# adahbingee/pais-mvs

Measured on AMD Instinct MI355X. Metric: refined+expanded patches/sec, higher is better.
Workload: dtype f64

## Files before the change

include/pais_hip.h:

```cpp
#ifndef PAIS_HIP_H
#define PAIS_HIP_H

#include <stdint.h>
#include <stddef.h>

#ifdef __cplusplus
extern "C" {
#endif

#define PAIS_MAX_LEVELS 16
#define PAIS_MAX_VIS    64
#define PAIS_MAX_PARTICLES 128

#define PAIS_TYPE_SEED   0
#define PAIS_TYPE_EXPAND 1

typedef struct pais_config {
    int32_t cellSize;
    int32_t patchRadius;
    int32_t patchSize;
    int32_t minCamNum;
    double  textureVariation;
    double  visibleCorrelation;
    double  minCorrelation;
// ... 92 lines not shown

int  pais_ctx_create(const pais_config *cfg, int num_cams, const pais_camera_desc *cams,
                     int device, uint64_t pso_seed, pais_ctx **out);
int  pais_ctx_set_config(pais_ctx *ctx, const pais_config *cfg);
int  pais_ctx_set_neighbor_radius(pais_ctx *ctx, double neighbor_radius);
void pais_ctx_destroy(pais_ctx *ctx);

int  pais_fitness_batch(pais_ctx *ctx, int n_states, const pais_patch_state *states,
                        int n_evals, const int32_t *state_index, const double *particles,
                        double *out);

#define PAIS_COST_OK          0
#define PAIS_COST_BACKFACING  1
#define PAIS_COST_OFF_IMAGE   2
#define PAIS_COST_WINDOW      3
#define PAIS_COST_OVERFLOW    4
#define PAIS_COST_ALL_MASKED  5
#define PAIS_PIX_COUNTED      0
#define PAIS_PIX_MASKED       1
#define PAIS_PIX_OVERFLOW     2
#define PAIS_PIX_NONE         3

typedef struct pais_cost_detail {
    double  fitness;
    double  sum_weight;
    double  sum_weighted_sad;
    double  pt[2];
    int32_t outcome, nx, ny;
    int32_t live_pixels;
    int32_t overflow_pixel;
    int32_t overflow_cam;
    int32_t ref_pos, _pad;
} pais_cost_detail;

int  pais_fitness_detail(pais_ctx *ctx, int n_states, const pais_patch_state *states,
                         int n_evals, const int32_t *state_index, const double *particles,
                         pais_cost_detail *out, double *weight, double *avg_sad, int8_t *pixel_code,
                         double *colour, double *homographies, int cam_stride);
int  pais_get_detail_stats(pais_ctx *ctx, double *kernel_ms, int64_t *launches, int64_t *evals, int reset);
size_t pais_sizeof_cost_detail(void);

int  pais_refine_batch(pais_ctx *ctx, int n, const pais_candidate *cands, pais_patch_result *out);
int  pais_refine_batch_view(pais_ctx *ctx, int n, const pais_candidate *cands, const pais_patch_result **view);
int  pais_refine_batch_begin(pais_ctx *ctx, int n, const pais_candidate *cands);
int  pais_refine_batch_end(pais_ctx *ctx, const pais_patch_result **view);

typedef struct pais_pso_run_info {
    double  range_l[3], range_u[3];
    double  init[3];
    double  ray[3];
    int32_t run;
    int32_t ref_cam, lod, num_cam;
    int32_t n_particles, max_iteration;
    int32_t iterations;
    int32_t _pad;
    int32_t cam_idx[PAIS_MAX_VIS];
} pais_pso_run_info;

typedef struct pais_pso_iter {
    double  gbest_fitness, gbest[3];
    double  iw;
    double  dispersion, velocity;
    int32_t g_idx, iteration, ended, _pad;
} pais_pso_iter;

int  pais_pso_trace_shape(pais_ctx *ctx, int n, const pais_candidate *cands, int *rows_per_run, int *particles_per_row);
int  pais_pso_trace(pais_ctx *ctx, int n, const pais_candidate *cands, int max_runs, pais_patch_result *out,
                    pais_pso_run_info *runs, pais_pso_iter *iters, double *particles);
int  pais_get_trace_stats(pais_ctx *ctx, double *kernel_ms, int64_t *launches, int64_t *evals, int reset);
size_t pais_sizeof_pso_run_info(void);
size_t pais_sizeof_pso_iter(void);

int  pais_refine_batch_open(pais_ctx *ctx, int n, const pais_candidate *cands, int iterations);
int  pais_refine_batch_enqueue(pais_ctx *ctx, int iterations);
int  pais_ctx_fork_lane(pais_ctx *parent, pais_ctx **lane);
int  pais_ctx_set_round_hint(pais_ctx *ctx, int n_round);

int  pais_refine_batch_device(pais_ctx *ctx, int n, const pais_candidate *d_cands,
                              pais_patch_result *d_out, int max_num_cam, int has_seeds);
size_t pais_record_wire_bytes(int max_num_cam);
int  pais_pack_records(int n, const pais_patch_result *recs, int max_num_cam, void *wire);
int  pais_unpack_records(int n, const void *wire, int max_num_cam, pais_patch_result *recs);
int  pais_pack_records_device(pais_ctx *ctx, int n, const pais_patch_result *d_recs, int max_num_cam, void *d_wire);

#define PAIS_WIRE_MAGIC 0x50414953u
#define PAIS_WIRE_RC_RING_RETRY 1
#define PAIS_WIRE_HEADER_BYTES 64
int  pais_refine_batch_device_async(pais_ctx *ctx, int n, const pais_candidate *d_cands,
                                    pais_patch_result *d_out, int max_num_cam, int has_seeds);
int  pais_wire_header_device(pais_ctx *ctx, int rank, int count, int host_rc, uint32_t user_word, void *d_header);
int  pais_ctx_batch_status(pais_ctx *ctx);

void *pais_ctx_stream(pais_ctx *ctx);
int  pais_ctx_synchronize(pais_ctx *ctx);

typedef struct pais_kernel_stats {
    double   pso_ms;
    double   begin_ms;
    double   after_ms;
    int64_t  pso_launches;
    int64_t  pso_evals;
    int64_t  pso_patches;
    double   pso_algorithmic_bytes;
    double   ncc_algorithmic_bytes;
    int64_t  ncc_tables;
    double   eval_ms;
    int64_t  eval_launches;
    double   eval2_ms;
    int64_t  eval2_launches;
    int64_t  eval2_evals;
    double   eval2_algorithmic_bytes;
    int64_t  tile_launches;
    double   eval2_busy_ms;
    int64_t  ring_launches;
    double   ring_ms;
    int64_t  ring_evals;
    double   ring_algorithmic_bytes;
    int64_t  ring_fallbacks;
} pais_kernel_stats;
int  pais_get_kernel_stats(pais_ctx *ctx, pais_kernel_stats *out, int reset);
int  pais_ctx_set_fine_timing(pais_ctx *ctx, int on);

int  pais_neighbor_count(pais_ctx *ctx, int n, const double *centers, double radius, int32_t *counts, double *kernel_ms);

typedef struct pais_view_state {
    double  center[3];
    double  normal[3];
    int32_t ref_cam, lod, num_cam, _pad;
    int32_t cam_idx[PAIS_MAX_VIS];
} pais_view_state;

#define PAIS_VIEW_KEEP         0
#define PAIS_VIEW_REGION       1
#define PAIS_VIEW_BACKFACING   2
#define PAIS_VIEW_CORRELATION  3
#define PAIS_VIEW_DROP_SAMPLE  1
#define PAIS_VIEW_DROP_MINCAM  2

typedef struct pais_view_result {
    double  correlation;
    double  region_ratio[PAIS_MAX_VIS];
    int32_t dropped, max_idx, num_kept, _pad;
    int32_t reason[PAIS_MAX_VIS];
    int32_t kept_idx[PAIS_MAX_VIS];
} pais_view_result;

int  pais_ncc_batch(pais_ctx *ctx, int n, const pais_view_state *states, pais_view_result *out, double *tables, int stride);
int  pais_get_ncc_stats(pais_ctx *ctx, double *kernel_ms, int64_t *launches, int64_t *states, int reset);
size_t pais_sizeof_view_state(void);
size_t pais_sizeof_view_result(void);

typedef struct pais_loaded_patch {
    double  center[3], normalS[2], fitness, correlation;
    int32_t num_cam, _pad;
    int32_t cam_idx[PAIS_MAX_VIS];
} pais_loaded_patch;
int  pais_load_state_batch(pais_ctx *ctx, int n, const pais_loaded_patch *in, pais_patch_result *out);
int  pais_get_load_stats(pais_ctx *ctx, double *kernel_ms, int64_t *launches, int64_t *patches, int reset);
size_t pais_sizeof_loaded_patch(void);

uint32_t pais_rand31(uint64_t seed, uint64_t key, uint32_t run, uint32_t k);
uint64_t pais_child_key(uint64_t parent_key, int cam, int cx, int cy);

const char *pais_last_error(void);
size_t pais_sizeof_config(void);
size_t pais_sizeof_camera_desc(void);
// ... 8 lines not shown
```

pais_mvs_amd/_lib.py:

```python
from __future__ import annotations

import ctypes as C
import os

from . import build as _build

MAX_LEVELS = 16
MAX_VIS = 64


class Config(C.Structure):
    _fields_ = [
        ("cellSize", C.c_int32), ("patchRadius", C.c_int32), ("patchSize", C.c_int32), ("minCamNum", C.c_int32),
        ("textureVariation", C.c_double), ("visibleCorrelation", C.c_double), ("minCorrelation", C.c_double),
        ("maxFitness", C.c_double), ("lodRatio", C.c_double),
        ("minLOD", C.c_int32), ("maxLOD", C.c_int32), ("maxCellPatchNum", C.c_int32), ("_pad0", C.c_int32),
        ("reduceNormalRange", C.c_double),
        ("adaptiveDistanceEnable", C.c_int32), ("adaptiveDifferenceEnable", C.c_int32),
        ("adaptiveGradientEnable", C.c_int32), ("_pad1", C.c_int32),
        ("distWeighting", C.c_double), ("diffWeighting", C.c_double), ("gradientWeighting", C.c_double),
        ("neighborRadius", C.c_double), ("neighborRadiusScalar", C.c_double), ("minRegionRatio", C.c_double),
        ("depthRangeScalar", C.c_double),
        ("particleNum", C.c_int32), ("maxIteration", C.c_int32), ("expansionStrategy", C.c_int32), ("_pad2", C.c_int32),
    ]
# ... 78 lines not shown
                ("velocity", C.c_double), ("g_idx", C.c_int32), ("iteration", C.c_int32), ("ended", C.c_int32), ("_pad", C.c_int32)]


class View(C.Structure):
    _fields_ = [("R", C.c_double * 9), ("T", C.c_double * 3), ("focal", C.c_double * 2), ("pp", C.c_double * 2)]


RENDER_DISC, RENDER_POINT, RENDER_CULL_BACK, RENDER_MAX_POINT_SIZE = 0, 1, 1, 64
CLOUD_MAX_K, KNN_SKIP_SAME_INDEX = 32, 1


class Lens(C.Structure):
    _fields_ = [("focal", C.c_double * 2), ("pp", C.c_double * 2), ("k", C.c_double), ("model", C.c_int32), ("_pad", C.c_int32)]


LENS_MEASURED_TO_IDEAL, LENS_IDEAL_TO_MEASURED = 0, 1


class KernelStats(C.Structure):
    _fields_ = [("pso_ms", C.c_double), ("begin_ms", C.c_double), ("after_ms", C.c_double),
                ("pso_launches", C.c_int64), ("pso_evals", C.c_int64), ("pso_patches", C.c_int64),
                ("pso_algorithmic_bytes", C.c_double), ("ncc_algorithmic_bytes", C.c_double),
                ("ncc_tables", C.c_int64), ("eval_ms", C.c_double), ("eval_launches", C.c_int64),
                ("eval2_ms", C.c_double), ("eval2_launches", C.c_int64), ("eval2_evals", C.c_int64),
                ("eval2_algorithmic_bytes", C.c_double), ("tile_launches", C.c_int64), ("eval2_busy_ms", C.c_double), ("ring_launches", C.c_int64),
                ("ring_ms", C.c_double), ("ring_evals", C.c_int64), ("ring_algorithmic_bytes", C.c_double), ("ring_fallbacks", C.c_int64)]


_lib = None


def load(build_if_needed: bool = True):
    global _lib
    if _lib is not None:
        return _lib
    path = os.environ.get("PAIS_LIB_PATH") or _build.LIB
    if path != _build.LIB:
        build_if_needed = False
    if int(os.environ.get("WORLD_SIZE", "1")) > 1 or os.environ.get("PAIS_NO_BUILD"):
        build_if_needed = False
    if build_if_needed and _build.needs_build():
        try:
            _build.build()
        except Exception as e:
            if not os.path.exists(path):
                raise RuntimeError("libpais_hip.so is missing and could not be built: %s" % e)
    if not os.path.exists(path):
        raise RuntimeError("libpais_hip.so not found at %s -- run `python -m pais_mvs_amd.build`" % path)
    L = C.CDLL(path)
    L.pais_last_error.restype = C.c_char_p
    for n in ("pais_sizeof_config", "pais_sizeof_camera_desc", "pais_sizeof_candidate", "pais_sizeof_patch_result",
              "pais_sizeof_view_state", "pais_sizeof_view_result", "pais_sizeof_cost_detail",
              "pais_sizeof_pso_run_info", "pais_sizeof_pso_iter", "pais_sizeof_loaded_patch"):
        getattr(L, n).restype = C.c_size_t
    assert L.pais_sizeof_config() == C.sizeof(Config), (L.pais_sizeof_config(), C.sizeof(Config))
    assert L.pais_sizeof_camera_desc() == C.sizeof(CameraDesc)
    assert L.pais_sizeof_candidate() == C.sizeof(Candidate)
    assert L.pais_sizeof_patch_result() == C.sizeof(PatchResult), (L.pais_sizeof_patch_result(), C.sizeof(PatchResult))
    assert L.pais_sizeof_view_state() == C.sizeof(ViewState), (L.pais_sizeof_view_state(), C.sizeof(ViewState))
    assert L.pais_sizeof_view_result() == C.sizeof(ViewResult), (L.pais_sizeof_view_result(), C.sizeof(ViewResult))
    assert L.pais_sizeof_cost_detail() == C.sizeof(CostDetail), (L.pais_sizeof_cost_detail(), C.sizeof(CostDetail))
    assert L.pais_sizeof_pso_run_info() == C.sizeof(PsoRunInfo), (L.pais_sizeof_pso_run_info(), C.sizeof(PsoRunInfo))
    assert L.pais_sizeof_pso_iter() == C.sizeof(PsoIter), (L.pais_sizeof_pso_iter(), C.sizeof(PsoIter))
    assert L.pais_sizeof_loaded_patch() == C.sizeof(LoadedPatch), (L.pais_sizeof_loaded_patch(), C.sizeof(LoadedPatch))
    L.pais_ctx_create.restype = C.c_int
    L.pais_ctx_create.argtypes = [C.POINTER(Config), C.c_int, C.POINTER(CameraDesc), C.c_int, C.c_uint64,
                                  C.POINTER(C.c_void_p)]
    L.pais_ctx_set_config.argtypes = [C.c_void_p, C.POINTER(Config)]
    L.pais_ctx_set_neighbor_radius.argtypes = [C.c_void_p, C.c_double]
    L.pais_ctx_destroy.argtypes = [C.c_void_p]
    L.pais_ctx_destroy.restype = None
    L.pais_ctx_stream.restype = C.c_void_p
    L.pais_ctx_stream.argtypes = [C.c_void_p]
    L.pais_ctx_synchronize.argtypes = [C.c_void_p]
    L.pais_fitness_batch.argtypes = [C.c_void_p, C.c_int, C.POINTER(PatchState), C.c_int, C.POINTER(C.c_int32),
                                     C.POINTER(C.c_double), C.POINTER(C.c_double)]
    L.pais_refine_batch.argtypes = [C.c_void_p, C.c_int, C.POINTER(Candidate), C.POINTER(PatchResult)]
    L.pais_refine_batch_device.argtypes = [C.c_void_p, C.c_int, C.c_void_p, C.c_void_p, C.c_int, C.c_int]
    L.pais_refine_batch_begin.argtypes = [C.c_void_p, C.c_int, C.POINTER(Candidate)]
    L.pais_refine_batch_open.argtypes = [C.c_void_p, C.c_int, C.POINTER(Candidate), C.c_int]
    L.pais_refine_batch_enqueue.argtypes = [C.c_void_p, C.c_int]
    L.pais_ctx_set_round_hint.argtypes = [C.c_void_p, C.c_int]
    L.pais_refine_batch_end.argtypes = [C.c_void_p, C.POINTER(C.POINTER(PatchResult))]
    L.pais_ctx_fork_lane.argtypes = [C.c_void_p, C.POINTER(C.c_void_p)]
    L.pais_get_kernel_stats.argtypes = [C.c_void_p, C.POINTER(KernelStats), C.c_int]
    L.pais_ctx_set_fine_timing.argtypes = [C.c_void_p, C.c_int]
    L.pais_neighbor_count.argtypes = [C.c_void_p, C.c_int, C.POINTER(C.c_double), C.c_double, C.POINTER(C.c_int32), C.POINTER(C.c_double)]
    L.pais_ncc_batch.argtypes = [C.c_void_p, C.c_int, C.POINTER(ViewState), C.POINTER(ViewResult), C.POINTER(C.c_double), C.c_int]
    L.pais_fitness_detail.argtypes = [C.c_void_p, C.c_int, C.POINTER(PatchState), C.c_int, C.POINTER(C.c_int32),
                                      C.POINTER(C.c_double), C.POINTER(CostDetail), C.POINTER(C.c_double), C.POINTER(C.c_double),
                                      C.POINTER(C.c_int8), C.POINTER(C.c_double), C.POINTER(C.c_double), C.c_int]
    L.pais_pso_trace.argtypes = [C.c_void_p, C.c_int, C.POINTER(Candidate), C.c_int, C.POINTER(PatchResult), C.c_void_p, C.c_void_p,
                                 C.POINTER(C.c_double)]
    L.pais_pso_trace_shape.argtypes = [C.c_void_p, C.c_int, C.POINTER(Candidate), C.POINTER(C.c_int), C.POINTER(C.c_int)]
    L.pais_get_trace_stats.argtypes = [C.c_void_p, C.POINTER(C.c_double), C.POINTER(C.c_int64), C.POINTER(C.c_int64), C.c_int]
    L.pais_get_detail_stats.argtypes = [C.c_void_p, C.POINTER(C.c_double), C.POINTER(C.c_int64), C.POINTER(C.c_int64), C.c_int]
    L.pais_get_ncc_stats.argtypes = [C.c_void_p, C.POINTER(C.c_double), C.POINTER(C.c_int64), C.POINTER(C.c_int64), C.c_int]
    L.pais_load_state_batch.argtypes = [C.c_void_p, C.c_int, C.POINTER(LoadedPatch), C.POINTER(PatchResult)]
    L.pais_get_load_stats.argtypes = [C.c_void_p, C.POINTER(C.c_double), C.POINTER(C.c_int64), C.POINTER(C.c_int64), C.c_int]
    L.pais_cloud_nearest.argtypes = [C.c_int, C.c_int, C.POINTER(C.c_double), C.c_int, C.POINTER(C.c_double),
                                     C.POINTER(C.c_int32), C.POINTER(C.c_double), C.POINTER(C.c_double)]
    L.pais_cloud_knn.argtypes = [C.c_int, C.c_int, C.c_int, C.c_int, C.POINTER(C.c_double), C.c_int, C.POINTER(C.c_double),
                                 C.POINTER(C.c_int32), C.POINTER(C.c_double), C.POINTER(C.c_double)]
    L.pais_cloud_outlier_rule.argtypes = [C.c_int, C.c_int, C.POINTER(C.c_int32), C.POINTER(C.c_double), C.c_double,
                                          C.POINTER(C.c_double), C.POINTER(C.c_double), C.POINTER(C.c_uint8)]
    L.pais_cloud_normals.argtypes = [C.c_int, C.POINTER(C.c_double), C.POINTER(C.c_double)]
    L.pais_cloud_launches.restype = C.c_int64
    L.pais_cloud_launches.argtypes = []
    L.pais_cloud_last_error.restype = C.c_char_p
    L.pais_sizeof_view.restype = C.c_size_t
    assert L.pais_sizeof_view() == C.sizeof(View), (L.pais_sizeof_view(), C.sizeof(View))
    L.pais_cloud_render.argtypes = [C.c_int, C.c_int, C.c_int, C.c_int, C.POINTER(C.c_double), C.POINTER(C.c_double),
                                    C.POINTER(C.c_double), C.c_double, C.c_int, C.POINTER(View), C.c_int, C.c_int,
                                    C.POINTER(C.c_double), C.POINTER(C.c_int32), C.POINTER(C.c_double)]
    L.pais_render_launches.restype = C.c_int64
    L.pais_render_launches.argtypes = []
    L.pais_render_last_error.restype = C.c_char_p
    L.pais_render_last_counts.restype = None
    L.pais_render_last_counts.argtypes = [C.POINTER(C.c_int64)] * 4
    L.pais_sizeof_lens.restype = C.c_size_t
    assert L.pais_sizeof_lens() == C.sizeof(Lens), (L.pais_sizeof_lens(), C.sizeof(Lens))
    for n in ("pais_undistort_points", "pais_distort_points"):
        getattr(L, n).argtypes = [C.c_int, C.POINTER(Lens), C.c_int64, C.POINTER(C.c_double), C.POINTER(C.c_double),
                                  C.POINTER(C.c_uint8), C.POINTER(C.c_double)]
    L.pais_undistort_image.argtypes = [C.c_int, C.POINTER(Lens), C.c_int, C.c_void_p, C.c_int, C.c_int, C.c_int64, C.c_void_p,
                                       C.c_void_p, C.POINTER(C.c_int64), C.POINTER(C.c_double)]
    L.pais_undistort_launches.restype = C.c_int64
    L.pais_undistort_launches.argtypes = []
    L.pais_undistort_last_error.restype = C.c_char_p
    L.pais_rand31.restype = C.c_uint32
    L.pais_rand31.argtypes = [C.c_uint64, C.c_uint64, C.c_uint32, C.c_uint32]
    L.pais_child_key.restype = C.c_uint64
    L.pais_child_key.argtypes = [C.c_uint64, C.c_int, C.c_int, C.c_int]
    _lib = L
    return L


def check(rc: int, what: str = ""):
    if rc != 0:
        raise RuntimeError("%s failed (%d): %s" % (what or "pais call", rc, load().pais_last_error().decode()))
```

pais_mvs_amd/context.py:

```python
from __future__ import annotations

import ctypes as C
import math
from typing import List, Sequence

import numpy as np

from . import _lib
from .camera import Camera
from .config import MvsConfig


def camera_desc(cam: Camera, with_edges: bool, keep: list) -> "_lib.CameraDesc":
    d = _lib.CameraDesc()
    d.focal[:] = list(map(float, cam.focal))
    d.principle_point[:] = list(map(float, cam.principle_point))
    d.rotation[:] = cam.rotation.ravel().tolist()
    d.translation[:] = cam.translation.tolist()
    d.center[:] = cam.center.tolist()
    d.KR[:] = cam.KR.ravel().tolist()
    d.KT[:] = cam.KT.tolist()
    d.optical_normal[:] = cam.optical_normal.tolist()
    d.max_lod = cam.max_lod
    for l, img in enumerate(cam.pyramid):
        img = np.ascontiguousarray(img, dtype=np.uint8)
        keep.append(img)
        d.level_width[l] = img.shape[1]
        d.level_height[l] = img.shape[0]
        d.level_stride[l] = img.strides[0]
        d.level_image[l] = img.ctypes.data
        if with_edges and cam.edge_pyramid:
            e = np.ascontiguousarray(cam.edge_pyramid[l], dtype=np.float64)
            keep.append(e)
            d.level_edge[l] = e.ctypes.data
    return d


def normal_to_spherical(n) -> List[float]:
    return [math.acos(float(n[2])), math.atan2(float(n[1]), float(n[0]))]


class Context:

    def __init__(self, cfg: MvsConfig, cameras: Sequence[Camera], device: int = 0, seed: int = 42):
        self.L = _lib.load()
        self.cfg = cfg
        self.cameras = list(cameras)
        self._keep: list = []
        n = len(self.cameras)
        descs = (_lib.CameraDesc * n)()
        for i, cam in enumerate(self.cameras):
            descs[i] = camera_desc(cam, bool(cfg.adaptiveGradientEnable), self._keep)
        self._c_cfg = cfg.to_c()
        h = C.c_void_p()
        _lib.check(self.L.pais_ctx_create(C.byref(self._c_cfg), n, descs, device, seed, C.byref(h)), "pais_ctx_create")
        self.h = h
        self._keep.clear()

    def close(self):
        if getattr(self, "h", None):
            self.L.pais_ctx_destroy(self.h)
            self.h = None

    def __del__(self):
        try:
            self.close()
        except Exception:
            pass

    def set_config(self, cfg: MvsConfig):
        c_cfg = cfg.to_c()
        _lib.check(self.L.pais_ctx_set_config(self.h, C.byref(c_cfg)), "pais_ctx_set_config")
        self.cfg = cfg
        self._c_cfg = c_cfg

    def set_neighbor_radius(self, r: float):
        _lib.check(self.L.pais_ctx_set_neighbor_radius(self.h, float(r)))

    def fitness_batch(self, states: Sequence["_lib.PatchState"], state_index: Sequence[int], particles) -> np.ndarray:
        ns = len(states)
        arr = (_lib.PatchState * ns)(*states)
        idx = np.ascontiguousarray(state_index, dtype=np.int32)
        pts = np.ascontiguousarray(particles, dtype=np.float64).reshape(-1, 3)
        assert len(idx) == len(pts)
        out = np.empty(len(idx), dtype=np.float64)
        _lib.check(self.L.pais_fitness_batch(self.h, ns, arr, len(idx), idx.ctypes.data_as(C.POINTER(C.c_int32)),
                                             pts.ctypes.data_as(C.POINTER(C.c_double)),
                                             out.ctypes.data_as(C.POINTER(C.c_double))), "pais_fitness_batch")
        return out

    def refine_batch(self, cands: Sequence["_lib.Candidate"]):
        n = len(cands)
        arr = (_lib.Candidate * n)(*cands)
        out = (_lib.PatchResult * n)()
        _lib.check(self.L.pais_refine_batch(self.h, n, arr, out), "pais_refine_batch")
        return out

    def ncc_batch(self, states: Sequence["_lib.ViewState"], tables: bool = False) -> "NccBatch":
        n = len(states)
        arr = (_lib.ViewState * max(n, 1))(*states)
        out = (_lib.ViewResult * max(n, 1))()
        stride = max([int(s.num_cam) for s in states] + [2])
        tab = np.zeros((n, stride, stride), dtype=np.float64) if tables else None
        tp = tab.ctypes.data_as(C.POINTER(C.c_double)) if tables else None
        _lib.check(self.L.pais_ncc_batch(self.h, n, arr, out, tp, stride), "pais_ncc_batch")
        return NccBatch([int(s.num_cam) for s in states], out, tab)

    def load_state_batch(self, patches: Sequence["_lib.LoadedPatch"]):
        n = len(patches)
        arr = (_lib.LoadedPatch * max(n, 1))(*patches)
        out = (_lib.PatchResult * max(n, 1))()
        _lib.check(self.L.pais_load_state_batch(self.h, n, arr, out), "pais_load_state_batch")
        return out

    def load_stats(self, reset: bool = False):
        ms, launches, np_ = C.c_double(), C.c_int64(), C.c_int64()
        _lib.check(self.L.pais_get_load_stats(self.h, C.byref(ms), C.byref(launches), C.byref(np_), 1 if reset else 0))
        return ms.value, launches.value, np_.value

    def fitness_detail(self, states: Sequence["_lib.PatchState"], state_index: Sequence[int], particles, colours: bool = False,
                       homographies: bool = False) -> "CostDetail":
        ns = len(states)
        arr = (_lib.PatchState * max(ns, 1))(*states)
        idx = np.ascontiguousarray(state_index, dtype=np.int32)
        pts = np.ascontiguousarray(particles, dtype=np.float64).reshape(-1, 3)
        assert len(idx) == len(pts)
        n, S = len(idx), int(self.cfg.patchSize)
        K = max([int(s.num_cam) for s in states] + [1])
        rec = (_lib.CostDetail * max(n, 1))()
        weight = np.zeros((n, S, S), dtype=np.float64)
        avg_sad = np.zeros((n, S, S), dtype=np.float64)
        code = np.zeros((n, S, S), dtype=np.int8)
        col = np.zeros((n, K, S, S), dtype=np.float64) if colours else None
        hom = np.zeros((n, K, 9), dtype=np.float64) if homographies else None
        dp = lambda a: a.ctypes.data_as(C.POINTER(C.c_double)) if a is not None else None
        _lib.check(self.L.pais_fitness_detail(self.h, ns, arr, n, idx.ctypes.data_as(C.POINTER(C.c_int32)), dp(pts), rec, dp(weight),
                                              dp(avg_sad), code.ctypes.data_as(C.POINTER(C.c_int8)), dp(col), dp(hom), K),
                   "pais_fitness_detail")
        num_cam = [int(states[i].num_cam) for i in idx.tolist()]
        return CostDetail(rec, n, weight, avg_sad, code, col, hom, num_cam, int(self.cfg.patchRadius))

    def pso_trace(self, cands: Sequence["_lib.Candidate"], max_runs: int = 1, particles: bool = False) -> "PsoTrace":
        n = len(cands)
        arr = (_lib.Candidate * max(n, 1))(*cands)
        rows, npart = C.c_int(0), C.c_int(0)
        _lib.check(self.L.pais_pso_trace_shape(self.h, n, arr, C.byref(rows), C.byref(npart)), "pais_pso_trace_shape")
        R, N = rows.value, npart.value
        out = (_lib.PatchResult * max(n, 1))()
        run_info = np.zeros((n, max(int(max_runs), 1)), dtype=PSO_RUN_INFO_DTYPE)
        iters = np.zeros((n, max(int(max_runs), 1), R), dtype=PSO_ITER_DTYPE)
        parts = np.zeros((n, max(int(max_runs), 1), R, N, 11), dtype=np.float64) if particles else None
        pp = parts.ctypes.data_as(C.POINTER(C.c_double)) if parts is not None else None
        _lib.check(self.L.pais_pso_trace(self.h, n, arr, int(max_runs), out, run_info.ctypes.data_as(C.c_void_p),
                                         iters.ctypes.data_as(C.c_void_p), pp), "pais_pso_trace")
        return PsoTrace(out, n, run_info, iters, parts)

    def trace_stats(self, reset: bool = False):
        ms, launches, ne = C.c_double(), C.c_int64(), C.c_int64()
        _lib.check(self.L.pais_get_trace_stats(self.h, C.byref(ms), C.byref(launches), C.byref(ne), 1 if reset else 0))
        return ms.value, launches.value, ne.value

    def detail_stats(self, reset: bool = False):
        ms, launches, ne = C.c_double(), C.c_int64(), C.c_int64()
        _lib.check(self.L.pais_get_detail_stats(self.h, C.byref(ms), C.byref(launches), C.byref(ne), 1 if reset else 0))
        return ms.value, launches.value, ne.value

    def ncc_stats(self, reset: bool = False):
        ms, launches, nst = C.c_double(), C.c_int64(), C.c_int64()
        _lib.check(self.L.pais_get_ncc_stats(self.h, C.byref(ms), C.byref(launches), C.byref(nst), 1 if reset else 0))
        return ms.value, launches.value, nst.value

    def kernel_stats(self, reset: bool = False) -> "_lib.KernelStats":
        st = _lib.KernelStats()
        _lib.check(self.L.pais_get_kernel_stats(self.h, C.byref(st), 1 if reset else 0))
        return st


def make_candidate(center, normal, cam_idx, key: int, ptype: int, normalS=None) -> "_lib.Candidate":
    c = _lib.Candidate()
    c.center[:] = [float(v) for v in center]
# ... 196 lines not shown
```

pais_mvs_amd/csrc/pais_capi.hip:

```cpp
#include <hip/hip_runtime.h>
#include <limits.h>
#include <math.h>
#include <stdarg.h>
#include <stddef.h>
#include <stdio.h>
#include <stdlib.h>
#include <string.h>

#include <string>
#include <utility>
#include <vector>
#include <algorithm>

#include "../../include/pais_hip.h"
#include "../../include/pais_test_hooks.h"
#include "pais_dev.hpp"
#include "pais_host.hpp"
#include "pais_internal.h"

static thread_local std::string g_err;
static int fail(const char *what, hipError_t e)
{
    char buf[512];
    snprintf(buf, sizeof(buf), "%s: %s", what, hipGetErrorString(e));
    g_err = buf;
    return -2;
}
static int fail_msg(const char *what)
{
    g_err = what;
    return -1;
}
__attribute__((format(printf, 1, 2))) static int fail_fmt(const char *fmt, ...)
{
    char buf[512];
    va_list ap;
    va_start(ap, fmt);
    vsnprintf(buf, sizeof(buf), fmt, ap);
    va_end(ap);
    return fail_msg(buf);
}
#define HIPCHK(call)                                   \
    do {                                               \
        hipError_t e__ = (call);                       \
        if (e__ != hipSuccess) return fail(#call, e__); \
    } while (0)

struct EventPair {
    hipEvent_t a, b;
};

struct pais_ctx;
struct Timed {
    pais_ctx *ctx = nullptr;
    hipStream_t st = nullptr;
    std::vector<EventPair> *into = nullptr;
    EventPair e{nullptr, nullptr};
    bool on = false;
    int begin(pais_ctx *c, hipStream_t s, std::vector<EventPair> *v);
    int end();
};
struct LaunchStats {
    double ms = 0;
    int64_t launches = 0, items = 0;
};
struct TimedLaunch {
    pais_ctx *ctx;
    EventPair e{nullptr, nullptr};
    explicit TimedLaunch(pais_ctx *c) : ctx(c) {}
    TimedLaunch(TimedLaunch &&o) noexcept : ctx(o.ctx), e(o.e) { o.e = EventPair{nullptr, nullptr}; }
    ~TimedLaunch();
    int begin();
    int end();
    void collect(LaunchStats &s, int64_t items, int64_t launches = 1);
};
struct TraceOut {
    pais_launch::TraceSink sink{nullptr, nullptr, nullptr, 1, 1};
    std::vector<TimedLaunch> passes;
    int64_t launches = 0;
};
struct PassPlan {
    struct Slice { int lo, hi, parts; pais_launch::BatchView v; pais_launch::TraceSink trace; };
    pais_launch::BatchView all{};
    int nSl = 0, S = 1, afterGrid = 0, itNext = 0;
    bool useIter = false, useTile = false, useRing = false, hasSeeds = false;
    bool usePre = false;
    int ringCUs = 0;
    Slice sl[16];
    int *cnt = nullptr, *nextCnt = nullptr;
    const pais_candidate *d_cands = nullptr;
    Timed tp;
    TraceOut *trace = nullptr;
};

struct pais_ctx {
    int device = 0;
    hipStream_t stream = nullptr;
    int numCUs = 256;
    size_t ldsLimit = 64 * 1024;
    DevScene sc;
    DevBuf<DevCamera> d_cams;
    DevBuf<uint8_t> d_img;
    DevBuf<PaisImgT> d_imgF;
    DevBuf<double> d_edge;
    bool edgesOnTheFly = false;
    DevBuf<double> d_gauss;
    size_t imgBytes = 0, edgeBytes = 0;
    std::vector<int> camMaxLod;
    DevBuf<pais_candidate> d_cands;
    DevBuf<pais_patch_result> d_recs;
    PinBuf<pais_candidate> h_cands;
    PinBuf<pais_patch_result> h_recs;
    DevBuf<double> d_hp;
    DevBuf<double> d_ratios;
    DevBuf<int> d_counters;
    unsigned passSerial = 0;
    bool countersDirty = false;
    DevBuf<unsigned char> d_evalBlocks;
    DevBuf<unsigned char> d_win;
    DevBuf<int> d_active;
    DevBuf<unsigned long long> d_stat;
    unsigned long long *stat = nullptr;
    PinBuf<int> h_counters;
    DevBuf<unsigned char> d_psoStates;
    long splitAbove = 0;
    int psoMinPer = 64;
    int evalParts = 0;
    double partFill = 0.5;
    int psoStreams = 2;
    pais_launch::TileOpts tile;
    int arithLiteral = 0;
    bool tileVerify = false;
    bool tileDebug = false;
    int tileMode = 1;
    long tileAbove = 512;
    std::vector<hipStream_t> sub;
    std::vector<hipEvent_t> subDone;
    hipEvent_t forkEv = nullptr;
    DevBuf<pais_patch_state> d_states;
    DevBuf<int32_t> d_idx;
    DevBuf<double> d_particles, d_out;
    DevBuf<pais_view_state> d_vStates;
    DevBuf<pais_view_result> d_vOut;
    DevBuf<double> d_vTables, d_vHp;
    LaunchStats ncc;
    DevBuf<pais_loaded_patch> d_lIn;
    DevBuf<pais_patch_result> d_lOut;
    LaunchStats load;
    DevBuf<pais_patch_state> d_dStates;
    DevBuf<int32_t> d_dIdx;
    DevBuf<double> d_dParticles, d_dWeight, d_dSad, d_dColour, d_dH;
    DevBuf<pais_cost_detail> d_dRec;
    DevBuf<int8_t> d_dCode;
    LaunchStats detail;
    DevBuf<pais_candidate> d_tCands;
    DevBuf<pais_patch_result> d_tRecs;
    DevBuf<pais_pso_run_info> d_tRuns;
    DevBuf<pais_pso_iter> d_tIters;
    DevBuf<double> d_tParts;
    DevBuf<unsigned long long> d_tStat;
    LaunchStats trace;
    DevBuf<double> d_nbC;
    DevBuf<int32_t> d_nbN;
    bool fineTiming = false;
    std::vector<EventPair> evPso, evBegin, evAfter, evEval, evEval2;
    std::vector<EventPair> evFree;
    double psoMs = 0, beginMs = 0, afterMs = 0, evalMs = 0, eval2Ms = 0;
    hipEvent_t refEv = nullptr;
    std::vector<std::pair<float, float>> eval2Intervals;
    int64_t psoLaunches = 0, evalLaunches = 0, eval2Launches = 0, tileLaunches = 0, ringLaunches = 0;
    pais_ctx *parent = nullptr;
    std::vector<pais_ctx *> lanes;
    int openBatch = -1;
    double ringPerCam = 1843.0;
    int ringMode = 1;
    int preMode = 1;
    DevBuf<double> d_pre;
    DevBuf<unsigned> d_ring;
    DevBuf<unsigned> d_ringCtl;
    PinBuf<unsigned> h_ringCtl;
    DevBuf<int> d_arrive;
    bool ringUsed = false;
    bool ringSuppressed = false;
    bool ringSuppressOnce = false;
    int ringPendingN = 0;
    double ringTimeoutMs = 10000.0;
    long ringSeedAbove = 0;
    size_t ringMaxBytes = (size_t)512 << 20;
    int64_t ringFallbacks = 0;
    std::vector<EventPair> evRing;
    double ringMs = 0;
    PassPlan plan;
    bool planDone = true;
    int roundHint = 0;
};
// ... 812 lines not shown
    if (itEnd > P.all.maxIt + 1) itEnd = P.all.maxIt + 1;
    if (P.useRing) {
        if (P.itNext == 0 && itEnd > 0) {
            const unsigned long long ticks = (unsigned long long)(ctx->ringTimeoutMs * 1e5);
            auto ring = [&](int phase) {
                return pais_launch::pso_ring(sc, P.all, ctx->d_ring, ctx->d_ringCtl, ctx->d_arrive, ctx->stat, P.ringCUs, phase, ticks);
            };
            HIPCHK(ring(0));
            Timed te;
            if (te.begin(ctx, ctx->stream, &ctx->evRing)) return -2;
            HIPCHK(ring(1));
            if (te.end()) return -2;
            HIPCHK(hipMemcpyAsync(ctx->h_ringCtl, ctx->d_ringCtl, PAIS_RING_CTL_BYTES * PAIS_RINGS, hipMemcpyDeviceToHost, ctx->stream));
            ctx->ringUsed = true;
            ctx->evalLaunches++;
            ctx->eval2Launches++;
            ctx->ringLaunches++;
            P.itNext = P.all.maxIt + 1;
        }
        return 0;
    }
    TimedLaunch tpass(ctx);
    const bool timePass = P.trace && itEnd > P.itNext;
    if (timePass && tpass.begin()) return -2;
    for (int it = P.itNext; it < itEnd; ++it) {
        for (int k = 0; k < P.nSl; ++k) {
            const PassPlan::Slice &q = P.sl[k];
            Timed te;
            if (te.begin(ctx, q.v.stream, P.useIter ? &ctx->evEval : &ctx->evEval2)) return -2;
            if (P.useIter)
                HIPCHK(pais_launch::pso_iter(sc, q.v, ctx->d_active, P.cnt + 2, q.lo, q.hi, ctx->stat, it, 0, q.parts));
            else if (P.useTile) {
                HIPCHK(pais_launch::pso_tile(sc, q.v, ctx->tile, ctx->tileDebug ? ctx->stat + 8 : nullptr));
                HIPCHK(pais_launch::pso_eval(sc, q.v, ctx->tileVerify ? 2 : 1, ctx->stat + 18));
            } else if (ctx->arithLiteral)
                HIPCHK(pais_launch::pso_eval_literal(sc, q.v));
            else
                HIPCHK(pais_launch::pso_eval(sc, q.v, 0, nullptr));
            if (te.end()) return -2;
            ctx->evalLaunches++;
            if (!P.useIter) ctx->eval2Launches++;
            if (P.useTile) ctx->tileLaunches++;
            if (P.trace) {
                HIPCHK(pais_launch::pso_step_trace(sc, q.v, ctx->stat, q.trace));
                P.trace->launches++;
            } else if (!P.useIter)
                HIPCHK(pais_launch::pso_step(sc, q.v, ctx->stat));
        }
    }
    if (timePass) {
        if (tpass.end()) return -2;
        P.trace->passes.push_back(std::move(tpass));
    }
    if (itEnd > P.itNext) P.itNext = itEnd;
    return 0;
}

static int pass_join(pais_ctx *ctx, PassPlan &P)
{
    for (int sI = 1; sI < P.S; ++sI) {
        bool used = false;
        for (int k = 0; k < P.nSl; ++k) used = used || (P.sl[k].v.stream == ctx->sub[sI - 1]);
        if (!used) continue;
        HIPCHK(hipEventRecord(ctx->subDone[sI - 1], ctx->sub[sI - 1]));
        HIPCHK(hipStreamWaitEvent(ctx->stream, ctx->subDone[sI - 1], 0));
    }
    P.S = 1;
    return 0;
}

static int pass_close(pais_ctx *ctx, PassPlan &P)
{
    const DevScene &sc = ctx->sc;
    for (int k = 0; k < P.nSl; ++k) {
        const PassPlan::Slice &q = P.sl[k];
        if (P.useIter)
            HIPCHK(pais_launch::pso_iter(sc, q.v, ctx->d_active, P.cnt + 2, q.lo, q.hi, ctx->stat, P.all.maxIt + 1, 1, q.parts));
    }
    if (pass_join(ctx, P)) return -2;
    if (P.tp.end()) return -2;
    ctx->psoLaunches++;
    Timed ta;
    if (ta.begin(ctx, ctx->stream, &ctx->evAfter)) return -2;
    HIPCHK(pais_launch::after(sc, P.all.recs, P.all.n, ctx->d_hp, P.afterGrid, P.cnt, ctx->stat, P.all.Kmax, ctx->d_ratios, P.nextCnt, ctx->stream));
    if (ta.end()) return -2;
    return 0;
}

static int batch_setup(pais_ctx *ctx, PassPlan &P, int n, const pais_candidate *d_cands, pais_patch_result *d_out, int max_num_cam, int has_seeds)
{
    HIPCHK(hipSetDevice(ctx->device));
    const DevScene &sc = ctx->sc;
    int Kmax = max_num_cam > 0 ? max_num_cam : sc.numCams;
    if (Kmax > PAIS_MAX_VIS) Kmax = PAIS_MAX_VIS;
    if (Kmax > sc.numCams) Kmax = sc.numCams;
    if (Kmax < 1) Kmax = 1;
    const int Nmax = has_seeds ? sc.cfg.particleNum * 2 : sc.cfg.particleNum;
    const int S2 = sc.cfg.patchSize * sc.cfg.patchSize;
    const int afterGrid = n < 2048 ? n : 2048;
    {
        size_t hpNeed = (size_t)afterGrid * Kmax * S2 * sizeof(double);
        const size_t full = (size_t)2048 * Kmax * S2 * sizeof(double);
        if (hpNeed > ctx->d_hp.bytes && full < ((size_t)1 << 31)) hpNeed = full;
        HIPCHK(ctx->d_hp.reserve(ctx->stream, hpNeed));
    }
    HIPCHK(ctx->d_active.reserve(ctx->stream, sizeof(int) * (size_t)n));
    HIPCHK(ctx->d_evalBlocks.reserve(ctx->stream, pais_launch::eval_block_bytes_host(Kmax) * (size_t)n));
    HIPCHK(ctx->d_win.reserve(ctx->stream, pais_launch::win_bytes_per_candidate(sc) * (size_t)n));
    HIPCHK(ctx->d_psoStates.reserve(ctx->stream, pais_launch::pso_state_bytes_host(Nmax) * (size_t)n));
    HIPCHK(ctx->d_ratios.reserve(ctx->stream, sizeof(double) * PAIS_MAX_VIS * (size_t)n));
    P.all = pais_launch::BatchView{d_out, ctx->d_psoStates, ctx->d_evalBlocks, ctx->d_win, nullptr, n, Nmax, Kmax,
                                   has_seeds ? sc.cfg.maxIteration * 2 : sc.cfg.maxIteration, ctx->stream};
    P.hasSeeds = has_seeds != 0;
    P.afterGrid = afterGrid;
    P.d_cands = d_cands;

    if (ctx->countersDirty) HIPCHK(hipMemsetAsync(ctx->d_counters, 0, sizeof(int) * 8, ctx->stream));
    ctx->countersDirty = true;
    Timed tb;
    if (tb.begin(ctx, ctx->stream, &ctx->evBegin)) return -2;
    HIPCHK(pais_launch::begin(sc, P.all, d_cands, ctx->d_active, ctx->d_counters + 4 * (ctx->passSerial & 1) + 2));
    if (tb.end()) return -2;
    return 0;
}

static int ring_failed(pais_ctx *ctx, int n)
{
    if (!ctx->ringUsed) return 0;
    ctx->ringUsed = false;
    unsigned done = 0, err = 0;
    for (int r = 0; r < PAIS_RINGS; ++r) { done += ctx->h_ringCtl[(PAIS_RING_CTL_BYTES / 4) * r + PAIS_RING_CTL_DONE_WORD]; err |= ctx->h_ringCtl[(PAIS_RING_CTL_BYTES / 4) * r + PAIS_RING_CTL_ERROR_WORD]; }
    if (err == 0 && done == (unsigned)n) return 0;
    ctx->ringFallbacks++;
    if (getenv("PAIS_RING_VERBOSE") || (ctx->ringFallbacks == 1 && ctx->ringTimeoutMs > 0))
        fprintf(stderr, "[pais] k_pso_ring did not complete (error %u, %u of %d runs ended): the batch is re-run with one launch per iteration\n", err, done, n);
    return 1;
}

static int refine_device_once(pais_ctx *ctx, int n, const pais_candidate *d_cands, pais_patch_result *d_out, int max_num_cam, int has_seeds,
                              bool defer = false, TraceOut *trace = nullptr)
{
    PassPlan &P = ctx->plan;
    P.trace = trace;
    ctx->ringUsed = false;
    ctx->ringPendingN = 0;
    int rc = batch_setup(ctx, P, n, d_cands, d_out, max_num_cam, has_seeds);
    int againCount = 0;
    const int maxPass = has_seeds ? (PAIS_MAX_VIS + 2) : 1;
    for (int pass = 0; !rc && pass < maxPass; ++pass) {
        if ((rc = pass_open(ctx, P, pass, againCount)) != 0) break;
        if ((rc = pass_iterations(ctx, P, P.all.maxIt + 1)) != 0) { (void)pass_join(ctx, P); break; }
        if ((rc = pass_close(ctx, P)) != 0) break;
        if (!has_seeds && !ctx->ringUsed) break;
        if (!has_seeds && defer) { ctx->ringPendingN = n; break; }
        if (has_seeds) HIPCHK(hipMemcpyAsync(ctx->h_counters, P.cnt, sizeof(int) * 2, hipMemcpyDeviceToHost, ctx->stream));
        HIPCHK(hipStreamSynchronize(ctx->stream));
        if (ring_failed(ctx, n)) { ctx->roundHint = 0; return 1; }
        if (!has_seeds || ctx->h_counters[1] == 0) break;
        againCount = ctx->h_counters[1];
    }
    ctx->roundHint = 0;
    if (rc) return rc;
    ctx->countersDirty = false;
    return 0;
}

static int rerun_without_ring(pais_ctx *ctx, int n, const pais_candidate *d_cands, pais_patch_result *d_out, int max_num_cam, int has_seeds,
                              bool defer, int hint)
{
    ctx->ringSuppressed = true;
    ctx->countersDirty = true;
    ctx->roundHint = hint;
    const int rc = refine_device_once(ctx, n, d_cands, d_out, max_num_cam, has_seeds, defer);
    ctx->ringSuppressed = false;
    return rc;
}

static int refine_device(pais_ctx *ctx, int n, const pais_candidate *d_cands, pais_patch_result *d_out, int max_num_cam, int has_seeds, bool defer)
{
    const int hint = ctx->roundHint;
    const int rc = refine_device_once(ctx, n, d_cands, d_out, max_num_cam, has_seeds, defer);
    return rc == 1 ? rerun_without_ring(ctx, n, d_cands, d_out, max_num_cam, has_seeds, defer, hint) : rc;
}

extern "C" int pais_refine_batch_device(pais_ctx *ctx, int n, const pais_candidate *d_cands, pais_patch_result *d_out,
                                        int max_num_cam, int has_seeds)
{
    if (!ctx || n < 0) return fail_msg("pais_refine_batch_device: bad argument");
    if (n == 0) return 0;
    if (!d_cands || !d_out) return fail_msg("pais_refine_batch_device: null pointer");
    if (ctx->openBatch >= 0) return fail_msg("pais_refine_batch_device: a batch is open on this context");
    return refine_device(ctx, n, d_cands, d_out, max_num_cam, has_seeds, false);
}

extern "C" int pais_refine_batch_device_async(pais_ctx *ctx, int n, const pais_candidate *d_cands, pais_patch_result *d_out,
                                              int max_num_cam, int has_seeds)
{
    if (!ctx || n < 0) return fail_msg("pais_refine_batch_device_async: bad argument");
    if (n == 0) return 0;
    if (!d_cands || !d_out) return fail_msg("pais_refine_batch_device_async: null pointer");
    if (ctx->openBatch >= 0) return fail_msg("pais_refine_batch_device_async: a batch is open on this context");
    if (ctx->ringSuppressOnce) {
        ctx->ringSuppressOnce = false;
        return rerun_without_ring(ctx, n, d_cands, d_out, max_num_cam, has_seeds, true, ctx->roundHint);
    }
    return refine_device(ctx, n, d_cands, d_out, max_num_cam, has_seeds, true);
}

extern "C" int pais_ctx_batch_status(pais_ctx *ctx)
{
    if (!ctx) return fail_msg("pais_ctx_batch_status: bad argument");
    if (ctx->ringPendingN <= 0) return 0;
    const int n = ctx->ringPendingN;
    ctx->ringPendingN = 0;
    ctx->countersDirty = false;
    if (!ring_failed(ctx, n)) return 0;
    ctx->countersDirty = true;
    ctx->ringSuppressOnce = true;
    return 1;
}

extern "C" int pais_wire_header_device(pais_ctx *ctx, int rank, int count, int host_rc, uint32_t user_word, void *d_header)
{
    if (!ctx || !d_header) return fail_msg("pais_wire_header_device: bad argument");
    HIPCHK(hipSetDevice(ctx->device));
    HIPCHK(pais_launch::wire_header(d_header, ctx->ringPendingN > 0 ? ctx->d_ringCtl : nullptr, ctx->ringPendingN, rank, count, host_rc, user_word, ctx->stream));
    return 0;
}

extern "C" int pais_test_swarm_step(int device, pais_test_swarm *s, double *swarm)
{
    hipError_t e = hipSetDevice(device);
    if (e != hipSuccess) return (int)e;
    return pais_launch::test_swarm_step(s, swarm);
}

extern "C" int pais_ctx_set_round_hint(pais_ctx *ctx, int n_round)
{
    if (!ctx) return fail_msg("pais_ctx_set_round_hint: bad argument");
    ctx->roundHint = n_round > 0 ? n_round : 0;
    return 0;
}

extern "C" int pais_refine_batch_view(pais_ctx *ctx, int n, const pais_candidate *cands, const pais_patch_result **view)
{
    if (!ctx || n < 0) return fail_msg("pais_refine_batch: bad argument");
    if (n == 0) return 0;
    if (!cands || !view) return fail_msg("pais_refine_batch: null pointer");
    int rc = pais_refine_batch_begin(ctx, n, cands);
    if (rc) return rc;
    return pais_refine_batch_end(ctx, view);
}

extern "C" int pais_refine_batch_begin(pais_ctx *ctx, int n, const pais_candidate *cands)
{
    int rc = pais_refine_batch_open(ctx, n, cands, 1 << 20);
    if (rc) return rc;
    rc = pais_refine_batch_enqueue(ctx, 0);
    return rc < 0 ? rc : 0;
}

extern "C" int pais_refine_batch_enqueue(pais_ctx *ctx, int iterations)
{
    if (!ctx) return fail_msg("pais_refine_batch_enqueue: bad argument");
    if (ctx->openBatch < 0) return fail_msg("pais_refine_batch_enqueue: no batch is open on this context");
    if (ctx->planDone) return 1;
    HIPCHK(hipSetDevice(ctx->device));
    PassPlan &P = ctx->plan;
    const int itEnd = iterations > 0 && iterations < P.all.maxIt + 1 - P.itNext ? P.itNext + iterations : P.all.maxIt + 1;
    int rc = pass_iterations(ctx, P, itEnd);
    if (!rc && P.itNext <= P.all.maxIt) return 0;
    if (!rc) rc = pass_close(ctx, P);
    if (rc) { (void)pass_join(ctx, P); ctx->openBatch = -1; ctx->ringUsed = false; return rc; }
    ctx->countersDirty = false;
    HIPCHK(hipMemcpyAsync(ctx->h_recs, ctx->d_recs, sizeof(pais_patch_result) * (size_t)ctx->openBatch, hipMemcpyDeviceToHost, ctx->stream));
    ctx->planDone = true;
    return 1;
}

extern "C" int pais_refine_batch_end(pais_ctx *ctx, const pais_patch_result **view)
{
    if (!ctx || !view) return fail_msg("pais_refine_batch_end: bad argument");
    if (ctx->openBatch < 0) return fail_msg("pais_refine_batch_end: no batch is open on this context");
    if (!ctx->planDone) {
        const int rc = pais_refine_batch_enqueue(ctx, 0);
        if (rc < 0) return rc;
    }
    ctx->openBatch = -1;
    HIPCHK(hipSetDevice(ctx->device));
    HIPCHK(hipStreamSynchronize(ctx->stream));
    if (ring_failed(ctx, ctx->plan.all.n)) {
        const int n = ctx->plan.all.n;
        const int rc = rerun_without_ring(ctx, n, ctx->d_cands, ctx->d_recs, ctx->plan.all.Kmax, 0, false, ctx->roundHint);
        if (rc) return rc;
        HIPCHK(hipMemcpyAsync(ctx->h_recs, ctx->d_recs, sizeof(pais_patch_result) * (size_t)n, hipMemcpyDeviceToHost, ctx->stream));
        HIPCHK(hipStreamSynchronize(ctx->stream));
    }
    *view = ctx->h_recs;
    return 0;
}

extern "C" int pais_refine_batch_open(pais_ctx *ctx, int n, const pais_candidate *cands, int iterations)
{
    if (!ctx || n <= 0 || !cands) return fail_msg("pais_refine_batch_begin: bad argument");
    if (ctx->openBatch >= 0) return fail_msg("pais_refine_batch_begin: a batch is open on this context already");
    HIPCHK(hipSetDevice(ctx->device));
    ctx->ringUsed = false;
    int Kmax = 1, hasSeeds = 0;
    int rc = check_candidates(ctx, "pais_refine_batch", n, cands, Kmax, hasSeeds);
    if (rc) return rc;
    HIPCHK(ctx->d_cands.reserve(ctx->stream, sizeof(pais_candidate) * (size_t)n));
    HIPCHK(ctx->d_recs.reserve(ctx->stream, sizeof(pais_patch_result) * (size_t)n));
    HIPCHK(ctx->h_cands.reserve(ctx->stream, sizeof(pais_candidate) * (size_t)n));
    HIPCHK(ctx->h_recs.reserve(ctx->stream, sizeof(pais_patch_result) * (size_t)n));
    memcpy(ctx->h_cands, cands, sizeof(pais_candidate) * (size_t)n);
    HIPCHK(hipMemcpyAsync(ctx->d_cands, ctx->h_cands, sizeof(pais_candidate) * (size_t)n, hipMemcpyHostToDevice, ctx->stream));
    if (hasSeeds) {
        rc = pais_refine_batch_device(ctx, n, ctx->d_cands, ctx->d_recs, Kmax, 1);
        if (rc) return rc;
        HIPCHK(hipMemcpyAsync(ctx->h_recs, ctx->d_recs, sizeof(pais_patch_result) * (size_t)n, hipMemcpyDeviceToHost, ctx->stream));
        ctx->openBatch = n;
        ctx->planDone = true;
        return 0;
    }
    PassPlan &P = ctx->plan;
    rc = batch_setup(ctx, P, n, ctx->d_cands, ctx->d_recs, Kmax, 0);
    if (!rc) rc = pass_open(ctx, P, 0, 0);
    ctx->roundHint = 0;
    if (!rc && (rc = pass_iterations(ctx, P, iterations > 0 ? iterations : 0)) != 0) (void)pass_join(ctx, P);
    if (rc) { ctx->ringUsed = false; return rc; }
    ctx->openBatch = n;
    ctx->planDone = false;
    return 0;
}

extern "C" int pais_refine_batch(pais_ctx *ctx, int n, const pais_candidate *cands, pais_patch_result *out)
{
    if (n > 0 && !out) return fail_msg("pais_refine_batch: null pointer");
    const pais_patch_result *view = nullptr;
    int rc = pais_refine_batch_view(ctx, n, cands, &view);
    if (rc || n <= 0) return rc;
    memcpy(out, view, sizeof(pais_patch_result) * (size_t)n);
    return 0;
}

extern "C" int pais_pso_trace_shape(pais_ctx *ctx, int n, const pais_candidate *cands, int *rows_per_run, int *particles_per_row)
{
    if (!ctx || n < 0 || !rows_per_run || !particles_per_row) return fail_msg("pais_pso_trace_shape: bad argument");
    if (n > 0 && !cands) return fail_msg("pais_pso_trace_shape: null pointer (cands)");
    int Kmax = 1, hasSeeds = 0;
    const int rc = check_candidates(ctx, "pais_pso_trace_shape", n, cands, Kmax, hasSeeds);
    if (rc) return rc;
    const pais_config &cfg = ctx->sc.cfg;
    *rows_per_run = (hasSeeds ? 2 * cfg.maxIteration : cfg.maxIteration) + 1;
    *particles_per_row = hasSeeds ? 2 * cfg.particleNum : cfg.particleNum;
    return 0;
}

struct TraceScope {
    pais_ctx *ctx;
    unsigned long long *stat;
    bool fine, ringUsed;
    int roundHint, ringPendingN;
    int64_t launches[6];
    explicit TraceScope(pais_ctx *c) : ctx(c)
    {
        stat = c->stat;
        c->stat = c->d_tStat;
        fine = c->fineTiming;
        c->fineTiming = false;
        ringUsed = c->ringUsed;
        ringPendingN = c->ringPendingN;
        roundHint = c->roundHint;
        c->roundHint = 0;
        const int64_t l[6] = {c->psoLaunches, c->evalLaunches, c->eval2Launches, c->tileLaunches, c->ringLaunches, c->ringFallbacks};
        memcpy(launches, l, sizeof(launches));
    }
    ~TraceScope()
    {
        ctx->stat = stat;
        ctx->fineTiming = fine;
        ctx->ringUsed = ringUsed;
        ctx->ringPendingN = ringPendingN;
        ctx->roundHint = roundHint;
        ctx->psoLaunches = launches[0];
        ctx->evalLaunches = launches[1];
        ctx->eval2Launches = launches[2];
        ctx->tileLaunches = launches[3];
        ctx->ringLaunches = launches[4];
        ctx->ringFallbacks = launches[5];
        ctx->plan.trace = nullptr;
    }
};

extern "C" int pais_pso_trace(pais_ctx *ctx, int n, const pais_candidate *cands, int max_runs, pais_patch_result *out,
                              pais_pso_run_info *runs, pais_pso_iter *iters, double *particles)
{
    if (n == 0) return 0;
    if (!ctx) return fail_msg("pais_pso_trace: null pointer (ctx)");
    if (n < 0) return fail_msg("pais_pso_trace: n < 0");
    const char *missing = !cands ? "cands" : !out ? "out" : !runs ? "runs" : !iters ? "iters" : nullptr;
    if (missing) return fail_fmt("pais_pso_trace: null pointer (%s)", missing);
    if (max_runs < 1) return fail_fmt("pais_pso_trace: max_runs %d < 1", max_runs);
    if (ctx->openBatch >= 0) return fail_msg("pais_pso_trace: a stepwise batch is open on this context (pais_refine_batch_open .. _end)");
    int Kmax = 1, hasSeeds = 0;
    int rc = check_candidates(ctx, "pais_pso_trace", n, cands, Kmax, hasSeeds);
    if (rc) return rc;
    HIPCHK(hipSetDevice(ctx->device));
    const pais_config &cfg = ctx->sc.cfg;
    const int rows = (hasSeeds ? 2 * cfg.maxIteration : cfg.maxIteration) + 1;
    const int NP = hasSeeds ? 2 * cfg.particleNum : cfg.particleNum;
    const size_t runRows = (size_t)max_runs * rows;
    const size_t perCand = sizeof(pais_candidate) + sizeof(pais_patch_result) + (size_t)max_runs * sizeof(pais_pso_run_info) +
                           runRows * sizeof(pais_pso_iter) + (particles ? runRows * NP * 11 * sizeof(double) : 0);
    const int chunk = staging_chunk("PAIS_TRACE_STAGING_MB", n, perCand);
    if (!ctx->d_tStat) {
        HIPCHK(ctx->d_tStat.alloc(sizeof(unsigned long long) * 24));
        HIPCHK(hipMemset(ctx->d_tStat, 0, sizeof(unsigned long long) * 24));
    }
    HIPCHK(ctx->d_tCands.reserve(ctx->stream, sizeof(pais_candidate) * (size_t)chunk));
    HIPCHK(ctx->d_tRecs.reserve(ctx->stream, sizeof(pais_patch_result) * (size_t)chunk));
    HIPCHK(ctx->d_tRuns.reserve(ctx->stream, sizeof(pais_pso_run_info) * (size_t)max_runs * chunk));
    HIPCHK(ctx->d_tIters.reserve(ctx->stream, sizeof(pais_pso_iter) * runRows * chunk));
    if (particles) HIPCHK(ctx->d_tParts.reserve(ctx->stream, sizeof(double) * 11 * runRows * NP * chunk));
    TraceScope scope(ctx);
    for (int c0 = 0; c0 < n; c0 += chunk) {
        const int m = std::min(chunk, n - c0);
        const size_t nRuns = (size_t)max_runs * m;
        HIPCHK(hipMemcpyAsync(ctx->d_tCands, cands + c0, sizeof(pais_candidate) * (size_t)m, hipMemcpyHostToDevice, ctx->stream));
        HIPCHK(hipMemsetAsync(ctx->d_tRuns, 0, sizeof(pais_pso_run_info) * nRuns, ctx->stream));
        HIPCHK(hipMemsetAsync(ctx->d_tIters, 0, sizeof(pais_pso_iter) * nRuns * rows, ctx->stream));
        if (particles) HIPCHK(hipMemsetAsync(ctx->d_tParts, 0, sizeof(double) * 11 * nRuns * rows * NP, ctx->stream));
        TraceOut t;
        t.sink = pais_launch::TraceSink{ctx->d_tRuns, ctx->d_tIters, particles ? ctx->d_tParts.p : nullptr, max_runs, rows};
        rc = refine_device_once(ctx, m, ctx->d_tCands, ctx->d_tRecs, Kmax, hasSeeds, false, &t);
        if (rc) {
            (void)hipStreamSynchronize(ctx->stream);
            return rc < 0 ? rc : fail_msg("pais_pso_trace: unexpected ring pass");
        }
        HIPCHK(hipMemcpyAsync(out + c0, ctx->d_tRecs, sizeof(pais_patch_result) * (size_t)m, hipMemcpyDeviceToHost, ctx->stream));
        HIPCHK(hipMemcpyAsync(runs + (size_t)max_runs * c0, ctx->d_tRuns, sizeof(pais_pso_run_info) * nRuns, hipMemcpyDeviceToHost, ctx->stream));
        HIPCHK(hipMemcpyAsync(iters + runRows * c0, ctx->d_tIters, sizeof(pais_pso_iter) * nRuns * rows, hipMemcpyDeviceToHost, ctx->stream));
        if (particles)
            HIPCHK(hipMemcpyAsync(particles + runRows * NP * 11 * c0, ctx->d_tParts, sizeof(double) * 11 * nRuns * rows * NP, hipMemcpyDeviceToHost,
                                  ctx->stream));
        HIPCHK(hipStreamSynchronize(ctx->stream));
        for (TimedLaunch &p : t.passes) p.collect(ctx->trace, 0, 0);
        ctx->trace.launches += t.launches;
        for (int i = 0; i < m; ++i) ctx->trace.items += out[c0 + i].pso_evals;
    }
    return 0;
}

extern "C" int pais_get_trace_stats(pais_ctx *ctx, double *kernel_ms, int64_t *launches, int64_t *evals, int reset)
{
    return read_launch_stats(ctx ? &ctx->trace : nullptr, "pais_get_trace_stats", kernel_ms, launches, evals, reset);
}

static_assert(offsetof(pais_patch_result, imgPoint) == 136 && offsetof(pais_patch_result, key) == 1160 &&
              offsetof(pais_patch_result, type) == 1168 && offsetof(pais_patch_result, cam_idx) == 1200 &&
              offsetof(pais_patch_result, stage) == 1456 && sizeof(pais_patch_result) == 1488, "pais_patch_result layout");
static inline int wire_kw(int max_num_cam)
{
    int k = max_num_cam < 1 ? 1 : (max_num_cam > PAIS_MAX_VIS ? PAIS_MAX_VIS : max_num_cam);
    return (k + 1) & ~1;
}
extern "C" size_t pais_record_wire_bytes(int max_num_cam) { return 208 + 20 * (size_t)wire_kw(max_num_cam); }
extern "C" int pais_pack_records(int n, const pais_patch_result *recs, int max_num_cam, void *wire)
{
    if (n < 0 || (n && (!recs || !wire))) return fail_msg("pais_pack_records: bad argument");
    const int Kw = wire_kw(max_num_cam);
    const size_t WB = pais_record_wire_bytes(max_num_cam);
    for (int i = 0; i < n; ++i) {
        const unsigned char *r = (const unsigned char *)&recs[i];
        unsigned char *w = (unsigned char *)wire + WB * (size_t)i;
        memcpy(w, r, 136);
        memcpy(w + 136, r + 1160, 8);
        memcpy(w + 144, r + 1168, 32);
        memcpy(w + 176, r + 1456, 32);
        memcpy(w + 208, r + 136, 16 * (size_t)Kw);
        memcpy(w + 208 + 16 * (size_t)Kw, r + 1200, 4 * (size_t)Kw);
    }
    return 0;
}
extern "C" int pais_unpack_records(int n, const void *wire, int max_num_cam, pais_patch_result *recs)
{
    if (n < 0 || (n && (!recs || !wire))) return fail_msg("pais_unpack_records: bad argument");
    const int Kw = wire_kw(max_num_cam);
    const size_t WB = pais_record_wire_bytes(max_num_cam);
    for (int i = 0; i < n; ++i) {
        unsigned char *r = (unsigned char *)&recs[i];
        const unsigned char *w = (const unsigned char *)wire + WB * (size_t)i;
        memset(r, 0, sizeof(pais_patch_result));
        memcpy(r, w, 136);
        memcpy(r + 1160, w + 136, 8);
        memcpy(r + 1168, w + 144, 32);
        memcpy(r + 1456, w + 176, 32);
        memcpy(r + 136, w + 208, 16 * (size_t)Kw);
        memcpy(r + 1200, w + 208 + 16 * (size_t)Kw, 4 * (size_t)Kw);
    }
    return 0;
}
extern "C" int pais_pack_records_device(pais_ctx *ctx, int n, const pais_patch_result *d_recs, int max_num_cam, void *d_wire)
{
    if (!ctx || n < 0 || (n && (!d_recs || !d_wire))) return fail_msg("pais_pack_records_device: bad argument");
    HIPCHK(hipSetDevice(ctx->device));
    HIPCHK(pais_launch::pack_records(d_recs, n, wire_kw(max_num_cam), d_wire, ctx->stream));
    return 0;
}

static int collect_stats(pais_ctx *ctx, unsigned long long *st)
{
    HIPCHK(hipStreamSynchronize(ctx->stream));
    if (drain_events(ctx, ctx->evPso, ctx->psoMs)) return -2;
    if (drain_events(ctx, ctx->evBegin, ctx->beginMs)) return -2;
    if (drain_events(ctx, ctx->evAfter, ctx->afterMs)) return -2;
    if (drain_events(ctx, ctx->evEval, ctx->evalMs)) return -2;
    const hipEvent_t ref = ctx->parent ? ctx->parent->refEv : ctx->refEv;
// ... 93 lines not shown
```

pais_mvs_amd/csrc/pais_internal.h:

```cpp
#pragma once
#include <hip/hip_runtime.h>
#include <stdint.h>

#include "../../include/pais_hip.h"

#define PAIS_STAGE_DONE  0
#define PAIS_STAGE_PSO   1
#define PAIS_STAGE_AFTER 2
#define PAIS_STAGE_AFTER2 3
#define PAIS_STAGE_AFTER2_KEEP 4
#define PAIS_STAGE_AFTER2_SAME 7

struct DevCamera {
    double KR[9], KT[3], R[9], T[3], C[3], optN[3], focal[2], pp[2];
    int maxLOD;
    int pad;
    int w[PAIS_MAX_LEVELS], h[PAIS_MAX_LEVELS];
    uint64_t imgOff[PAIS_MAX_LEVELS];
    uint64_t edgeOff[PAIS_MAX_LEVELS];
    double edgeMin[PAIS_MAX_LEVELS], edgeMax[PAIS_MAX_LEVELS];
};

typedef float2 PaisImgT;

struct DevScene {
    pais_config cfg;
    const DevCamera *cams;
    const uint8_t *imgBlob;
    const PaisImgT *imgF;
    const double *edgeBlob;
    const double *gauss;
    double lodScale[PAIS_MAX_LEVELS];
    uint64_t seed;
    int numCams;
    int pad;
};

#ifndef PAIS_RINGS
#define PAIS_RINGS 8
#endif
#ifndef PAIS_ARRIVE_STRIDE
#define PAIS_ARRIVE_STRIDE 16
#endif
#define PAIS_RING_CTL_BYTES 128
#define PAIS_RING_CTL_DONE_WORD 17
#define PAIS_RING_CTL_ERROR_WORD 19

struct pais_test_swarm;
namespace pais_launch {
struct BatchView {
    pais_patch_result *recs;
    unsigned char *states;
    unsigned char *evalBlocks;
    unsigned char *win;
    double *pre;
    int n, Nmax, Kmax, maxIt;
    hipStream_t stream;
    BatchView slice(const DevScene &sc, int lo, int hi, hipStream_t st) const;
};
struct TraceSink {
    pais_pso_run_info *runs;
    pais_pso_iter *iters;
    double *particles;
    int maxRuns, rows;
};
struct TileOpts {
    int stripSteps = 16;
    int noTiles = 0;
};

size_t eval_block_bytes_host(int Kmax);
size_t win_bytes_per_candidate(const DevScene &sc);
size_t pso_state_bytes_host(int Nmax);
size_t pre_bytes_per_candidate(int Nmax, int Kmax);
hipError_t state_blocks(const DevScene &sc, const pais_patch_state *states, int nStates, int Kmax, unsigned char *evalBlocks, void *win,
                        hipStream_t stream);
hipError_t fitness(const DevScene &sc, const pais_patch_state *states, int nStates, const int32_t *idx, const double *particles,
                   double *out, int nEvals, int Kmax, unsigned char *evalBlocks, void *win, int literal, hipStream_t stream);
hipError_t fitness_detail(const DevScene &sc, const int32_t *idx, const double *particles, int nEvals, int Kmax, const unsigned char *evalBlocks,
                          pais_cost_detail *rec, double *weight, double *avgSad, int8_t *code, double *colour, double *H, hipStream_t stream);
hipError_t load_state(const DevScene &sc, const pais_loaded_patch *in, pais_patch_result *recs, int n, uint64_t key0, hipStream_t stream);
hipError_t neighbor_count(const double *centers, int n, double radius, int32_t *counts, hipStream_t stream);
hipError_t expand_image(const uint8_t *img, PaisImgT *out, size_t n, hipStream_t stream);
hipError_t level_edge_minmax(const uint8_t *img, int w, int h, unsigned long long *minmax, hipStream_t stream);
hipError_t pack_records(const pais_patch_result *recs, int n, int Kw, void *wire, hipStream_t stream);
hipError_t wire_header(void *header, const unsigned *ringCtl, int ringN, int rank, int count, int hostRc, uint32_t userWord, hipStream_t stream);

hipError_t begin(const DevScene &sc, const BatchView &v, const pais_candidate *cands, int *activeList, int *activeCount);
hipError_t pso_init(const DevScene &sc, const BatchView &v, int *activeList, int *activeCount);
hipError_t pso_setup0(const DevScene &sc, const BatchView &v);
hipError_t pso_eval(const DevScene &sc, const BatchView &v, int pendingOnly, unsigned long long *verify);
hipError_t pso_eval_literal(const DevScene &sc, const BatchView &v);
bool tile_eligible(int Kmax);
hipError_t pso_tile(const DevScene &sc, const BatchView &v, const TileOpts &o, unsigned long long *dbg);
hipError_t pso_iter(const DevScene &sc, const BatchView &v, const int *activeList, const int *activeCount, int listLo, int listHi,
                    unsigned long long *stat, int L, int finishOnly, int nparts);
hipError_t pso_step(const DevScene &sc, const BatchView &v, unsigned long long *stat);
hipError_t pso_step_trace(const DevScene &sc, const BatchView &v, unsigned long long *stat, const TraceSink &t);
size_t ring_words(int n, int Nmax, int maxIt);
bool pre_ring_ok(int Kmax);
hipError_t pso_ring(const DevScene &sc, const BatchView &v, unsigned *ring, unsigned *ctl, int *arrive, unsigned long long *stat, int waves,
                    int phase, unsigned long long timeoutTicks);
void ring_profile_print();
hipError_t after(const DevScene &sc, pais_patch_result *recs, int n, double *hpScratch, int grid, int *counters,
                 unsigned long long *stat, int Kmax, double *ratios, int *nextCounters, hipStream_t stream);
size_t ncc_lds_bytes(int Kmax);
bool hp_in_lds(const DevScene &sc, int Kmax);
hipError_t ncc_batch(const DevScene &sc, const pais_view_state *states, int n, pais_view_result *out, double *tables, int stride,
                     double *hpScratch, int grid, int Kmax, int hpInLds, hipStream_t stream);
int test_swarm_step(pais_test_swarm *s, double *swarm);
}
```

pais_mvs_amd/csrc/pais_kernels.hip:

```cpp
#include <hip/hip_runtime.h>
#include <stdint.h>
#include <stdlib.h>
#include <string.h>

#include "../../include/pais_hip.h"
#include "../../include/pais_test_hooks.h"
#include "pais_dev.hpp"
#include "pais_internal.h"

using namespace pais;

#ifndef PAIS_NS1_WAVES
#define PAIS_NS1_WAVES 2
#endif
#ifndef PAIS_NS2_WAVES
#define PAIS_NS2_WAVES 3
#endif
#define PAIS_EVAL_BOUNDS(NS) __launch_bounds__(64, (NS) == 1 ? PAIS_NS1_WAVES : PAIS_NS2_WAVES)
#ifndef PAIS_ITER_FREE_REGS_FROM
#define PAIS_ITER_FREE_REGS_FROM 2
#endif
#define PAIS_ITER_BOUNDS(P, NS) __launch_bounds__(64, (P) >= PAIS_ITER_FREE_REGS_FROM ? 1 : ((NS) == 1 ? PAIS_NS1_WAVES : PAIS_NS2_WAVES))
#ifndef PAIS_TWO_PIXELS_MAXK
#define PAIS_TWO_PIXELS_MAXK 6
// ... 1871 lines not shown
        }
        const uint64_t v0 = lane < nwMax ? src[lane] : 0, v1 = lane + 64 < nwMax ? src[lane + 64] : 0;
        const int N = hd->N;
        wave_sync();
        stage_eval_block(smem, src, nwMax, lane, v0, v1);
        wave_sync();
#if PAIS_RING_PROFILE
        asm volatile("s_waitcnt vmcnt(0)" ::: "memory");
#endif
        PAIS_RP_MARK(rpD)
        double f4[4], w4[4];
        int st;
        if (PRE) st = eval_fitness_pre<NS, BYTES, ACCR, true>(sc, ep, cams, Hbuf, cbuf, win + (size_t)c * WS, rec, status0, hv, lane, f4, w4);
        else st = eval_fitness_parts<NS, BYTES, ACCR>(sc, ep, cams, Hbuf, cbuf, win + (size_t)c * WS, p0, p1, p2, lane, 0, 1, f4, w4);
        int old = 0;
        PAIS_RP_MARK(rpE)
        if (lane == 0) {
            cstore(&A.fit[i], st ? DBL_MAX : combine_parts(f4, w4));
            asm volatile("s_waitcnt vmcnt(0)" ::: "memory");
            old = __hip_atomic_fetch_add(&arrive[(size_t)c * PAIS_ARRIVE_STRIDE], 1, __ATOMIC_RELAXED, __HIP_MEMORY_SCOPE_AGENT);
        }
        old = __builtin_amdgcn_readfirstlane(old);
#if PAIS_RING_PROFILE
        {
            const unsigned long long rpF = __builtin_amdgcn_s_memtime();
            if (lane == 0) {
                atomicAdd(&g_ringProf[0], rpB - rpA); atomicAdd(&g_ringProf[1], rpC - rpB); atomicAdd(&g_ringProf[2], rpD - rpC);
                atomicAdd(&g_ringProf[3], rpE - rpD); atomicAdd(&g_ringProf[4], rpF - rpE); atomicAdd(&g_ringProf[6], 1ULL);
            }
        }
        PAIS_RP_MARK(rpG)
#endif
        if (old != N - 1) continue;
        __builtin_amdgcn_s_setprio(3);
        if (lane == 0) cstore(&arrive[(size_t)c * PAIS_ARRIVE_STRIDE], 0);
        wave_sync();
        const int cont = pso_step_wave_ring(sc, recs, c, hd, __builtin_amdgcn_readfirstlane(N), Nmax, smem + (PRE ? eval_block_bytes(Kmax) : 0), stat, lane, ep, cams, crec, preD);
        asm volatile("s_waitcnt vmcnt(0)" ::: "memory");
        wave_sync();
        if (__builtin_amdgcn_readfirstlane(cont)) {
            unsigned base = 0;
            if (lane == 0) base = __hip_atomic_fetch_add(&ctl->tail, (unsigned)N, __ATOMIC_RELAXED, __HIP_MEMORY_SCOPE_AGENT);
            base = (unsigned)__builtin_amdgcn_readfirstlane((int)base);
            if (base + (unsigned)N > cap) {
                if (lane == 0) rstore(&ctl->error, 2u);
                break;
            }
            if (lane < N) rstore(&ring[base + lane], ((unsigned)c << 8) | (unsigned)lane);
        } else if (lane == 0) {
            __hip_atomic_fetch_add(&ctl->done, 1u, __ATOMIC_RELAXED, __HIP_MEMORY_SCOPE_AGENT);
        }
        __builtin_amdgcn_s_setprio(0);
#if PAIS_RING_PROFILE
        {
            const unsigned long long rpH = __builtin_amdgcn_s_memtime();
            if (lane == 0) { atomicAdd(&g_ringProf[5], rpH - rpG); atomicAdd(&g_ringProf[7], 1ULL); }
        }
#endif
    }
}

__global__ __launch_bounds__(64) void k_region_ratio(DevScene sc, const pais_patch_result *recs, int n, int stage, double *ratios, int Kmax)
{
    const int t = blockIdx.x * 64 + threadIdx.x;
    const int c = t / Kmax, k = t - c * Kmax;
    if (c >= n) return;
    const pais_patch_result *P = &recs[c];
    if (P->stage != stage || P->dropped || k >= P->num_cam) return;
    const int LOD = P->lod, refCam = P->ref_cam;
    const DevCamera &rc = sc.cams[refCam];
    const double s = sc.lodScale[LOD];
    const double center[3] = {P->center[0], P->center[1], P->center[2]};
    const double nrm[3] = {P->normal[0], P->normal[1], P->normal[2]};
    const int ci = P->cam_idx[k];
    const double d = -dot3(center, nrm);
    double invH[9], H[9];
    ref_plane_inverse(d, s, rc.KR, rc.KT, nrm, invH);
    patch_homography(ci == refCam, d, s, sc.cams[ci].KR, sc.cams[ci].KT, nrm, invH, H);
    double pt[2];
    cam_project(sc, refCam, center, pt, LOD);
    ratios[(size_t)c * PAIS_MAX_VIS + k] = region_ratio(pt[0], pt[1], sc.cfg.patchRadius, H);
}

template <int PHASE>
__global__ __launch_bounds__(64 * AFTER_WAVES) void k_after(DevScene sc, pais_patch_result *recs, int n, double *hpScratch,
                                                              int *counters, unsigned long long *stat, int Kmax, double *ratios,
                                                              int hpInLds, int *nextCounters)
{
    if (PHASE == 2 && nextCounters && blockIdx.x == 0 && threadIdx.x == 0) {
        nextCounters[0] = 0;
        nextCounters[1] = 0;
        nextCounters[2] = 0;
    }
    extern __shared__ __attribute__((aligned(16))) unsigned char smem[];
    pais_patch_result *st = (pais_patch_result *)smem;
    size_t off = (sizeof(pais_patch_result) + 15) & ~(size_t)15;
    double *table = (double *)(smem + off); off += sizeof(double) * Kmax * Kmax;
    double *Hn = (double *)(smem + off); off += sizeof(double) * 9 * Kmax;
    int *flag = (int *)(smem + off); off += 16;
    const int lane = threadIdx.x & 63, wave = threadIdx.x >> 6;
    const bool lead = threadIdx.x == 0;
    const int S2 = sc.cfg.patchSize * sc.cfg.patchSize;
    double *hp = hpInLds ? (double *)(smem + off) : hpScratch + (size_t)blockIdx.x * Kmax * S2;
    for (int c = blockIdx.x; c < n; c += gridDim.x) {
        const int stg = recs[c].stage;
        if (PHASE == 1 ? (stg != PAIS_STAGE_AFTER) : (stg != PAIS_STAGE_AFTER2 && stg != PAIS_STAGE_AFTER2_KEEP && stg != PAIS_STAGE_AFTER2_SAME))
            continue;
        __syncthreads();
        copy_record(st, &recs[c], threadIdx.x, 64 * AFTER_WAVES);
        __syncthreads();

        const int nccBefore = st->ncc_tables;
        double *rat = ratios + (size_t)c * PAIS_MAX_VIS;
        if (PHASE == 1) {
            const int refBefore = st->ref_cam, lodBefore = st->lod, numBefore = st->num_cam;
            remove_invisible_camera(sc, st, hp, table, Hn, flag, rat, lane, wave);
            const bool removedNone = st->num_cam == numBefore;
            set_reference_camera(sc, st, lane);
            set_depth_and_ray(sc, st, lane);
            set_depth_range(sc, st, lane);
            set_lod(sc, st, lane);

            bool again = false;
            if (st->type != PAIS_TYPE_EXPAND && !st->dropped) {
                const int afterRef = st->ref_cam, afterNum = st->num_cam;
                const int cnt = st->count;
                const bool cond = (st->before_ref != afterRef || st->before_num != afterNum) && (cnt <= st->total_cam_num);
                __syncthreads();
                if (lead) {
                    st->after_ref = afterRef;
                    st->after_num = afterNum;
                    st->count = cnt + 1;
                }
                __syncthreads();
                if (cond) {
                    if (st->num_cam < sc.cfg.minCamNum) {
                        __syncthreads();
                        if (lead) {
                            st->fitness = DBL_MAX;
                            st->priority = DBL_MAX;
                            st->dropped = 1;
                        }
                        __syncthreads();
                    } else {
                        again = true;
                        __syncthreads();
                        if (lead) {
                            st->before_ref = st->ref_cam;
                            st->before_num = st->num_cam;
                            st->stage = PAIS_STAGE_PSO;
                        }
                        __syncthreads();
                    }
                }
            }
            if (!again) {
                set_priority_and_image_point(sc, st, lane);
                __syncthreads();
                if (lead)
                    st->stage = st->dropped ? PAIS_STAGE_DONE
                                            : ((st->ref_cam == refBefore && st->lod == lodBefore)
                                                   ? (removedNone ? PAIS_STAGE_AFTER2_SAME : PAIS_STAGE_AFTER2_KEEP)
                                                   : PAIS_STAGE_AFTER2);
            }
            __syncthreads();
            if (lead && again) atomicAdd(&counters[1], 1);
        } else {
            if (stg == PAIS_STAGE_AFTER2_SAME) {
                if (lead) st->ncc_tables += 1;
            } else {
                remove_invisible_camera(sc, st, hp, table, Hn, flag, rat, lane, wave);
            }
            __syncthreads();
            int finalStage = PAIS_DONE;
            if (!st->dropped) {
                bool off = false;
                const double X[3] = {st->center[0], st->center[1], st->center[2]};
                for (int i = threadIdx.x; i < sc.numCams; i += 64 * AFTER_WAVES) {
                    const DevCamera &cam = sc.cams[i];
                    double pt[2];
                    project_raw(cam.R, cam.T, cam.focal, cam.pp, 1.0, X, pt);
                    if (!in_image_d(pt, cam.w[0], cam.h[0])) {
                        off = true;
                    } else {
                        const int rx = min(cv_round(pt[0]), cam.w[0] - 1), ry = min(cv_round(pt[1]), cam.h[0] - 1);
                        if (sc.imgBlob[cam.imgOff[0] + (size_t)ry * cam.w[0] + rx] == 0) off = true;
                    }
                }
                finalStage = __syncthreads_or(off ? 1 : 0) ? PAIS_DONE_OFF_SCENE : PAIS_DONE_IN_SCENE;
            }
            if (lead) st->stage = finalStage;
        }
        __syncthreads();
        if (lead) {
            atomicAdd(&stat[3], (unsigned long long)(st->ncc_tables - nccBefore));
            atomicAdd(&stat[4], (unsigned long long)(st->ncc_tables - nccBefore) * (unsigned long long)st->total_cam_num);
        }
        __syncthreads();
        copy_record(&recs[c], st, threadIdx.x, 64 * AFTER_WAVES);
    }
}

__global__ __launch_bounds__(64 * AFTER_WAVES) void k_ncc_batch(DevScene sc, const pais_view_state *states, int n,
                                                                  pais_view_result *out, double *tables, int stride,
                                                                  double *hpScratch, int Kmax, int hpInLds)
{
    extern __shared__ __attribute__((aligned(16))) unsigned char smem[];
    pais_view_result *res = (pais_view_result *)smem;
    size_t off = (sizeof(pais_view_result) + 15) & ~(size_t)15;
    double *table = (double *)(smem + off); off += sizeof(double) * Kmax * Kmax;
    double *Hn = (double *)(smem + off); off += sizeof(double) * 9 * Kmax;
    int *flag = (int *)(smem + off); off += 16;
    const int tid = threadIdx.x, lane = tid & 63, wave = tid >> 6;
    const int r = sc.cfg.patchRadius, S = sc.cfg.patchSize, S2 = S * S;
    double *hp = hpInLds ? (double *)(smem + off) : hpScratch + (size_t)blockIdx.x * Kmax * S2;
    for (int s = blockIdx.x; s < n; s += gridDim.x) {
        const pais_view_state *V = &states[s];
        const int K = V->num_cam, LOD = V->lod, refCam = V->ref_cam;
        const double center[3] = {V->center[0], V->center[1], V->center[2]};
        const double nrm[3] = {V->normal[0], V->normal[1], V->normal[2]};
        __syncthreads();
        {
            uint32_t *w = (uint32_t *)res;
            for (int i = tid; i < (int)(sizeof(pais_view_result) / 4); i += 64 * AFTER_WAVES) w[i] = 0;
        }
        for (int i = tid; i < K * K; i += 64 * AFTER_WAVES) table[i] = 0;
        if (tid == 0) *flag = 0;
        if (wave == 0) view_homographies(sc, refCam, sc.lodScale[LOD], V->cam_idx, K, center, nrm, Hn, lane);
        __syncthreads();

        double pt[2];
        cam_project(sc, refCam, center, pt, LOD);
        if (wave == AFTER_WAVES - 1)
            for (int c = lane; c < K; c += 64) res->region_ratio[c] = region_ratio(pt[0], pt[1], r, Hn + 9 * c);

        view_warp_patches(sc, V->cam_idx, K, LOD, Hn, pt[0] - r, pt[1] - r, hp, flag, lane, wave);
        __syncthreads();
        const bool dropSample = *flag != 0;
        if (!dropSample) view_fill_table(hp, K, S2, table, lane, wave);
        __syncthreads();
        if (tid == 0) {
            if (dropSample) {
                res->dropped = PAIS_VIEW_DROP_SAMPLE;
            } else {
                double correlation = 0;
                for (int i = 0; i < K; ++i)
                    for (int j = 0; j < K; ++j) correlation += table[i * K + j];
                correlation /= (double)(K * K - K);
                double maxCorr = -DBL_MAX;
                int maxIdx = 0;
                for (int i = 0; i < K; ++i) {
                    double corrSum = 0;
                    for (int j = 0; j < K; ++j) corrSum += table[i * K + j];
                    if (corrSum >= maxCorr) {
                        maxIdx = i;
                        maxCorr = corrSum;
                    }
                }
                int nn = 0;
                for (int i = 0; i < K; ++i) {
                    const int ci = V->cam_idx[i];
                    const DevCamera &cam = sc.cams[ci];
                    const double dd = nrm[0] * (-cam.optN[0]) + nrm[1] * (-cam.optN[1]) + nrm[2] * (-cam.optN[2]);
                    int why = PAIS_VIEW_KEEP;
                    if (res->region_ratio[i] < sc.cfg.minRegionRatio) why = PAIS_VIEW_REGION;
                    else if (dd < 0) why = PAIS_VIEW_BACKFACING;
                    else if (i != maxIdx && table[maxIdx * K + i] < sc.cfg.minCorrelation) why = PAIS_VIEW_CORRELATION;
                    res->reason[i] = why;
                    if (why == PAIS_VIEW_KEEP) res->kept_idx[nn++] = ci;
                }
                res->correlation = correlation;
                res->max_idx = maxIdx;
                res->num_kept = nn;
                res->dropped = nn < sc.cfg.minCamNum ? PAIS_VIEW_DROP_MINCAM : 0;
            }
        }
        if (tables) {
            double *T = tables + (size_t)s * stride * stride;
            for (int i = tid; i < stride * stride; i += 64 * AFTER_WAVES) {
                const int a = i / stride, b = i - a * stride;
                T[i] = (a < K && b < K) ? table[a * K + b] : 0.0;
            }
        }
        __syncthreads();
        {
            const uint32_t *src = (const uint32_t *)res;
            uint32_t *dst = (uint32_t *)&out[s];
            for (int i = tid; i < (int)(sizeof(pais_view_result) / 4); i += 64 * AFTER_WAVES) dst[i] = src[i];
        }
    }
}

__global__ __launch_bounds__(256) void k_pack_records(const pais_patch_result *recs, int n, int Kw, uint32_t *wire)
{
    const int wordsPerSlot = 52 + 5 * Kw;
    for (size_t t = (size_t)blockIdx.x * 256 + threadIdx.x; t < (size_t)n * wordsPerSlot; t += (size_t)gridDim.x * 256) {
        const int r = (int)(t / wordsPerSlot), w = (int)(t - (size_t)r * wordsPerSlot);
        const uint32_t *src = (const uint32_t *)&recs[r];
        int sw;
        if (w < 34) sw = w;
        else if (w < 36) sw = 290 + (w - 34);
        else if (w < 44) sw = 292 + (w - 36);
        else if (w < 52) sw = 364 + (w - 44);
        else if (w < 52 + 4 * Kw) sw = 34 + (w - 52);
        else sw = 300 + (w - 52 - 4 * Kw);
        wire[t] = src[sw];
    }
}

__global__ __launch_bounds__(64) void k_wire_header(uint32_t *hdr, const RingCtl *ctl, int ringN, int rank, int count, int hostRc, uint32_t userWord)
{
    if (threadIdx.x >= 16) return;
    int rc = hostRc;
    if (rc == 0 && ctl) {
        unsigned done = 0, err = 0;
        for (int r = 0; r < PAIS_RINGS; ++r) { done += ctl[r].done; err |= ctl[r].error; }
        if (err != 0 || done != (unsigned)ringN) rc = PAIS_WIRE_RC_RING_RETRY;
    }
    const uint32_t w[4] = {PAIS_WIRE_MAGIC, (uint32_t)rc, (uint32_t)count, (uint32_t)rank};
    hdr[threadIdx.x] = threadIdx.x < 4 ? w[threadIdx.x] : (threadIdx.x == 4 ? userWord : 0u);
}

__global__ __launch_bounds__(256) void k_expand_image(const uint8_t *img, PaisImgT *out, size_t n)
{
    for (size_t i = (size_t)blockIdx.x * 256 + threadIdx.x; i < n; i += (size_t)gridDim.x * 256) {
        const int a = img[i], b = (i + 1 < n) ? img[i + 1] : 0;
        PaisImgT v;
        v.x = a;
        v.y = b - a;
        out[i] = v;
    }
}
__global__ __launch_bounds__(256) void k_level_edge_minmax(const uint8_t *img, int w, int h, unsigned long long *minmax)
{
    __shared__ unsigned long long red[8];
    const int x = blockIdx.x * 256 + threadIdx.x;
    unsigned long long lo = ~0ULL, hi = 0ULL;
    if (x < w) {
        const int xl = x > 0 ? x - 1 : (w > 1 ? 1 : 0), xr = x < w - 1 ? x + 1 : (w > 1 ? w - 2 : 0);
        for (int r = 0; r < 16; ++r) {
            const int y = blockIdx.y * 16 + r;
            if (y >= h) break;
            const int yu = y > 0 ? y - 1 : (h > 1 ? 1 : 0), yd = y < h - 1 ? y + 1 : (h > 1 ? h - 2 : 0);
            const double gx = (double)img[(size_t)y * w + xr] - (double)img[(size_t)y * w + xl];
            const double gy = (double)img[(size_t)yd * w + x] - (double)img[(size_t)yu * w + x];
            const unsigned long long u = (unsigned long long)__double_as_longlong(sqrt(gx * gx + gy * gy));
            lo = u < lo ? u : lo;
            hi = u > hi ? u : hi;
        }
    }
    for (int s = 32; s >= 1; s >>= 1) {
        const unsigned long long ol = __shfl_xor(lo, s, 64), oh = __shfl_xor(hi, s, 64);
        lo = ol < lo ? ol : lo;
        hi = oh > hi ? oh : hi;
    }
    const int wave = threadIdx.x >> 6;
    if ((threadIdx.x & 63) == 0) {
        red[wave] = lo;
        red[4 + wave] = hi;
    }
    __syncthreads();
    if (threadIdx.x == 0) {
        for (int q = 1; q < 4; ++q) {
            lo = red[q] < lo ? red[q] : lo;
            hi = red[4 + q] > hi ? red[4 + q] : hi;
        }
        if (lo != ~0ULL) atomicMin(&minmax[0], lo);
        atomicMax(&minmax[1], hi);
    }
}

__global__ __launch_bounds__(256) void k_neighbor_count(const double *centers, int n, double radius, int32_t *counts)
{
    __shared__ double tile[256 * 3];
    const int i = blockIdx.x * 256 + threadIdx.x;
    const bool has = i < n;
    const double cx = has ? centers[3 * i] : 0, cy = has ? centers[3 * i + 1] : 0, cz = has ? centers[3 * i + 2] : 0;
    int cnt = 0;
    for (int base = 0; base < n; base += 256) {
        const int m = (n - base) < 256 ? (n - base) : 256;
        __syncthreads();
        for (int t = threadIdx.x; t < 3 * m; t += 256) tile[t] = centers[3 * (size_t)base + t];
        __syncthreads();
        for (int j = 0; j < m; ++j) {
            const double dx = cx - tile[3 * j], dy = cy - tile[3 * j + 1], dz = cz - tile[3 * j + 2];
            double s2 = 0;
            s2 += dx * dx;
            s2 += dy * dy;
// ... 182 lines not shown
    const int groups = (v.Nmax + TILE2_SLOTS - 1) / TILE2_SLOTS;
    return launch<k_pso_tile2<NP>>(grid_for((long)v.n * groups, 65536), dim3(64 * TILE2_WAVES), lds, v.stream, sc, v.states, v.n, v.Nmax, v.Kmax,
                                   (const unsigned char *)v.evalBlocks, eval_block_bytes(v.Kmax), (const WinPix *)v.win,
                                   o.noTiles ? 0 : (int)(lds - fixed), groups, o.stripSteps, dbg);
}
hipError_t pso_tile(const DevScene &sc, const BatchView &v, const TileOpts &o, unsigned long long *dbg)
{
    if (v.Kmax <= 28) return tile_launch<8>(sc, v, o, dbg);
    if (v.Kmax <= 44) return tile_launch<12>(sc, v, o, dbg);
    return tile_launch<16>(sc, v, o, dbg);
}
hipError_t pso_iter(const DevScene &sc, const BatchView &v, const int *activeList, const int *activeCount, int listLo, int listHi,
                    unsigned long long *stat, int L, int finishOnly, int nparts)
{
    if (listHi <= listLo) return hipSuccess;
    return shape_dispatch(sc, v.Kmax, [&](auto ns, auto bytes, auto accr) {
        constexpr int NS = ns;
        constexpr bool BYTES = bytes, ACCR = accr;
        auto go = [&](auto parts) {
            return launch<k_pso_iter<parts, NS, BYTES, ACCR>>(grid_for((long)(listHi - listLo) * (finishOnly ? 1 : v.Nmax * parts), EVAL_GRID_CAP),
                                                              dim3(64), eval_lds_bytes(NS, v.Kmax, ACCR), v.stream, sc, v.states, activeList, activeCount,
                                                              listLo, listHi, v.Nmax, v.Kmax, v.recs, stat, L, finishOnly,
                                                              (const unsigned char *)v.evalBlocks, eval_block_bytes(v.Kmax), (const WinPix *)v.win);
        };
        return nparts == 4 ? go(Int<4>()) : (nparts == 2 ? go(Int<2>()) : go(Int<1>()));
    });
}
static size_t ring_seg_words(int n, int Nmax, int maxIt) { return (size_t)((n + PAIS_RINGS - 1) / PAIS_RINGS) * Nmax * ((size_t)maxIt + 2); }
size_t ring_words(int n, int Nmax, int maxIt) { return ring_seg_words(n, Nmax, maxIt) * PAIS_RINGS; }
hipError_t pso_ring(const DevScene &sc, const BatchView &v, unsigned *ring, unsigned *ctl, int *arrive, unsigned long long *stat, int waves,
                    int phase, unsigned long long timeoutTicks)
{
    const int n = v.n, Nmax = v.Nmax, Kmax = v.Kmax;
    if (Nmax > 64) return hipErrorInvalidValue;
    const size_t words = ring_words(n, Nmax, v.maxIt), seg = ring_seg_words(n, Nmax, v.maxIt);
    if (seg >= 0xFFFFFFF0ull) return hipErrorInvalidValue;
    if (phase == 0) {
        hipError_t e = hipMemsetAsync(ring, 0xFF, words * sizeof(unsigned), v.stream);
        if (e != hipSuccess) return e;
        e = hipMemsetAsync(ctl, 0, sizeof(RingCtl) * PAIS_RINGS, v.stream);
        if (e != hipSuccess) return e;
        e = hipMemsetAsync(arrive, 0, sizeof(int) * PAIS_ARRIVE_STRIDE * (size_t)n, v.stream);
        if (e != hipSuccess) return e;
        return launch<k_ring_init>(dim3((n + 255) / 256), dim3(256), 0, v.stream, v.states, n, Nmax, ring, (unsigned)seg, (RingCtl *)ctl);
    }
    return shape_dispatch(sc, Kmax, [&](auto ns, auto bytes, auto accr) {
        constexpr int NS = ns;
        constexpr bool BYTES = bytes, ACCR = accr;
        const size_t stepBytes = v.pre ? eval_block_bytes(Kmax) + step_lds_bytes(Nmax) : sizeof(double) * (size_t)Nmax * (3 * 4 + 2) + 16;
        size_t per = eval_lds_bytes(NS, Kmax, ACCR);
        if (per < stepBytes) per = stepBytes;
        per = (per + 15) & ~(size_t)15;
        const long resident = (long)waves * (NS == 1 ? 4 * PAIS_NS1_WAVES : 4 * PAIS_NS2_WAVES);
        const unsigned grid = (grid_for((long)n * Nmax, resident) + PAIS_RINGS - 1) / PAIS_RINGS * PAIS_RINGS;
        auto go = [&](auto usePre) {
            return launch<k_pso_ring<NS, BYTES, ACCR, usePre>>(dim3(grid), dim3(64), per, v.stream, sc, v.recs, v.states, n, Nmax, Kmax,
                                                               (const unsigned char *)v.evalBlocks, eval_block_bytes(Kmax), (const WinPix *)v.win, ring,
                                                               (unsigned)seg, (RingCtl *)ctl, arrive, stat, per, timeoutTicks, v.pre);
        };
        return v.pre ? go(Bool<true>()) : go(Bool<false>());
    });
}
hipError_t pso_step(const DevScene &sc, const BatchView &v, unsigned long long *stat)
{
    const size_t lds = v.pre ? eval_block_bytes(v.Kmax) + step_lds_bytes(v.Nmax) : sizeof(double) * (size_t)v.Nmax * (3 * 4 + 2);
    return launch<k_pso_step>(grid_for(v.n, 65536), dim3(64), lds, v.stream, sc, v.recs, v.states, v.n, v.Nmax, stat,
                              (const unsigned char *)v.evalBlocks, eval_block_bytes(v.Kmax), v.pre, v.Kmax);
}
hipError_t pso_step_trace(const DevScene &sc, const BatchView &v, unsigned long long *stat, const TraceSink &t)
{
    if (v.n <= 0) return hipSuccess;
    StepTraceSink sink;
    sink.runs = t.runs;
    sink.iters = t.iters;
    sink.particles = t.particles;
    sink.maxRuns = t.maxRuns;
    sink.rows = t.rows;
    sink.NP = v.Nmax;
    return launch<k_pso_step_trace>(grid_for(v.n, 65536), dim3(64), sizeof(double) * (size_t)v.Nmax * (3 * 4 + 2), v.stream, sc, v.recs, v.states,
                                    v.n, v.Nmax, stat, sink);
}

hipError_t after(const DevScene &sc, pais_patch_result *recs, int n, double *hpScratch, int grid, int *counters,
                 unsigned long long *stat, int Kmax, double *ratios, int *nextCounters, hipStream_t stream)
{
    if (n <= 0) return hipSuccess;
    const int hpInLds = hp_in_lds(sc, Kmax) ? 1 : 0;
    const size_t lds = ncc_scratch_bytes(sizeof(pais_patch_result), Kmax) + (hpInLds ? hp_bytes(sc, Kmax) : 0);
    const dim3 rgrid((unsigned)(((long)n * Kmax + 63) / 64)), block(64 * AFTER_WAVES);
    hipError_t e = launch<k_region_ratio>(rgrid, dim3(64), 0, stream, sc, recs, n, PAIS_STAGE_AFTER, ratios, Kmax);
    if (e == hipSuccess)
        e = launch<k_after<1>>(dim3(grid), block, lds, stream, sc, recs, n, hpScratch, counters, stat, Kmax, ratios, hpInLds, (int *)nullptr);
    if (e == hipSuccess) e = launch<k_region_ratio>(rgrid, dim3(64), 0, stream, sc, recs, n, PAIS_STAGE_AFTER2, ratios, Kmax);
    if (e == hipSuccess)
        e = launch<k_after<2>>(dim3(grid), block, lds, stream, sc, recs, n, hpScratch, counters, stat, Kmax, ratios, hpInLds, nextCounters);
    return e;
}
hipError_t ncc_batch(const DevScene &sc, const pais_view_state *states, int n, pais_view_result *out, double *tables, int stride,
                     double *hpScratch, int grid, int Kmax, int hpInLds, hipStream_t stream)
{
    if (n <= 0) return hipSuccess;
    const size_t lds = ncc_lds_bytes(Kmax) + (hpInLds ? hp_bytes(sc, Kmax) : 0);
    return launch<k_ncc_batch>(dim3(grid), dim3(64 * AFTER_WAVES), lds, stream, sc, states, n, out, tables, stride, hpScratch, Kmax, hpInLds);
}

__global__ __launch_bounds__(64) void k_test_swarm_step(DevScene sc, pais_patch_result *recs, unsigned char *states, int Nmax,
                                                        unsigned long long *stat, int *continues)
{
    extern __shared__ __attribute__((aligned(16))) unsigned char smem0[];
    PsoState *hd = (PsoState *)states;
    const int N = __builtin_amdgcn_readfirstlane(hd->N);
    const int cont = pso_step_wave(sc, recs, 0, hd, N, Nmax, smem0, stat, (int)threadIdx.x);
    if (threadIdx.x == 0) *continues = cont;
}
int test_swarm_step(pais_test_swarm *s, double *swarm)
{
    if (!s || !swarm || s->n < 1 || s->n > 128) return (int)hipErrorInvalidValue;
    const int N = s->n;
    const size_t SB = pso_state_bytes(N), head = (sizeof(PsoState) + 15) & ~(size_t)15;
    unsigned char *host = (unsigned char *)calloc(1, SB);
    if (!host) return (int)hipErrorOutOfMemory;
    PsoState *hd = (PsoState *)host;
    for (int d = 0; d < 3; ++d) {
        hd->rangeL[d] = s->range_l[d];
        hd->rangeU[d] = s->range_u[d];
        hd->ray[d] = d == 2 ? 1.0 : 0.0;
    }
    hd->iw = s->iw;
    hd->gBestFitness = s->gbest_fitness;
    hd->streamBase = s->stream_base;
    hd->gIdx = s->g_idx;
    hd->N = N;
    hd->maxIt = s->max_iteration;
    hd->iteration = s->iteration;
    hd->active = 1;
    hd->run = s->run;
    hd->localK = s->local_k;
    hd->started = s->started;
    hd->K = 3;
    double *arr = (double *)(host + head);
    for (int i = 0; i < N; ++i) {
        for (int a = 0; a < 4; ++a)
            for (int d = 0; d < 3; ++d) arr[(size_t)a * 3 * N + 3 * i + d] = swarm[14 * i + 3 * a + d];
        arr[(size_t)12 * N + i] = swarm[14 * i + 12];
        arr[(size_t)13 * N + i] = swarm[14 * i + 13];
    }
    unsigned char *dev = nullptr;
    const size_t offRec = (SB + 255) & ~(size_t)255, offStat = offRec + ((sizeof(pais_patch_result) + 255) & ~(size_t)255),
                 offCam = offStat + 256, offCont = offCam + ((sizeof(DevCamera) + 255) & ~(size_t)255), total = offCont + 256;
    hipError_t e = hipMalloc((void **)&dev, total);
    if (e == hipSuccess) e = hipMemset(dev, 0, total);
    if (e == hipSuccess) e = hipMemcpy(dev, host, SB, hipMemcpyHostToDevice);
    pais_patch_result rec;
    int cont = 0;
    if (e == hipSuccess) {
        DevScene sc;
        memset(&sc, 0, sizeof(sc));
        sc.cams = (const DevCamera *)(dev + offCam);
        sc.cfg.maxFitness = 10.0;
        sc.numCams = 1;
        e = launch<k_test_swarm_step>(dim3(1), dim3(64), sizeof(double) * (size_t)N * (3 * 4 + 2) + 16, nullptr, sc,
                                      (pais_patch_result *)(dev + offRec), dev, N, (unsigned long long *)(dev + offStat), (int *)(dev + offCont));
    }
    if (e == hipSuccess) e = hipDeviceSynchronize();
    if (e == hipSuccess) e = hipMemcpy(host, dev, SB, hipMemcpyDeviceToHost);
    if (e == hipSuccess) e = hipMemcpy(&rec, dev + offRec, sizeof(rec), hipMemcpyDeviceToHost);
    if (e == hipSuccess) e = hipMemcpy(&cont, dev + offCont, sizeof(int), hipMemcpyDeviceToHost);
    if (e == hipSuccess) {
        for (int i = 0; i < N; ++i) {
            for (int a = 0; a < 4; ++a)
                for (int d = 0; d < 3; ++d) swarm[14 * i + 3 * a + d] = arr[(size_t)a * 3 * N + 3 * i + d];
            swarm[14 * i + 12] = arr[(size_t)12 * N + i];
            swarm[14 * i + 13] = arr[(size_t)13 * N + i];
        }
        s->iw = hd->iw;
        s->gbest_fitness = hd->gBestFitness;
        s->g_idx = hd->gIdx;
        s->iteration = hd->iteration;
// ... 29 lines not shown
```

pais_mvs_amd/csrc/pais_mvs.hip:

```cpp
#include <float.h>
#include <limits.h>
#include <math.h>
#include <stdio.h>
#include <stdlib.h>
#include <string.h>

#include <algorithm>
#include <chrono>
#include <deque>
#include <queue>
#include <new>
#include <string>
#include <unordered_map>
#include <unordered_set>
#include <vector>

#include <dlfcn.h>
#include <hip/hip_runtime.h>

#include "../../include/pais_mvs.h"
#include "../../include/pais_test_hooks.h"
#include "../../include/pais_seed.h"
#include "../../include/pais_feature.h"
#include "../../include/pais_cloud.h"
// ... 780 lines not shown
        for (int i = 0; i < num_cam; i++) {
            const HostCamera &cam = m->cams[cam_idx[i]];
            for (int k = 0; k < 3; ++k) dir[k] = cam.C[k] - center[k];
            double sc = (1.0 / pais::norm3(dir));
            for (int k = 0; k < 3; ++k) dir[k] *= sc;
            for (int k = 0; k < 3; ++k) normal[k] += dir[k];
        }
        double sc = (1.0 / pais::norm3(normal));
        for (int k = 0; k < 3; ++k) r.normal[k] = normal[k] * sc;
        pais::normal2spherical(r.normal, r.normalS);
    } else {
        r.dropped = 1;
    }
    return m->storePatch(r);
}

extern "C" int pais_mvs_add_seed_measured(pais_mvs *m, const double center[3], int num_cam, const int32_t *cam_idx,
                                          const double *img_points, int recenter)
{
    if (!m || !center || num_cam < 0 || num_cam > PAIS_MAX_VIS || (num_cam && (!cam_idx || !img_points)))
        return mfail("pais_mvs_add_seed_measured: bad argument");
    for (int i = 0; i < num_cam; ++i)
        if (cam_idx[i] < 0 || cam_idx[i] >= (int)m->cams.size()) return mfail("pais_mvs_add_seed_measured: bad camera index");
    double c[3] = {center[0], center[1], center[2]};
    if (recenter) {
        double A[3][3] = {{0, 0, 0}, {0, 0, 0}, {0, 0, 0}}, b[3] = {0, 0, 0};
        for (int i = 0; i < num_cam; ++i) {
            const HostCamera &cam = m->cams[cam_idx[i]];
            const double p3[3] = {(img_points[2 * i] - cam.pp[0]) / cam.focal[0] - cam.T[0],
                                  (img_points[2 * i + 1] - cam.pp[1]) / cam.focal[1] - cam.T[1], 1.0 - cam.T[2]};
            double w3[3];
            for (int r = 0; r < 3; ++r) {
                double sacc = 0;
                for (int k = 0; k < 3; ++k) sacc += cam.R[k * 3 + r] * p3[k];
                w3[r] = sacc;
            }
            double n[3] = {w3[0] - cam.C[0], w3[1] - cam.C[1], w3[2] - cam.C[2]};
            const double sc = (1.0 / pais::norm3(n));
            for (int k = 0; k < 3; ++k) n[k] = n[k] * sc;
            const double *cc = cam.C;
            A[0][0] += 1 - n[0] * n[0];
            A[0][1] += -n[0] * n[1];
            A[0][2] += -n[0] * n[2];
            A[1][0] += -n[0] * n[1];
            A[1][1] += 1 - n[1] * n[1];
            A[1][2] += -n[1] * n[2];
            A[2][0] += -n[0] * n[2];
            A[2][1] += -n[1] * n[2];
            A[2][2] += 1 - n[2] * n[2];
            b[0] += (1 - n[0] * n[0]) * cc[0] - n[0] * n[1] * cc[1] - n[0] * n[2] * cc[2];
            b[1] += -n[0] * n[1] * cc[0] + (1 - n[1] * n[1]) * cc[1] - n[1] * n[2] * cc[2];
            b[2] += -n[0] * n[2] * cc[0] - n[1] * n[2] * cc[1] + (1 - n[2] * n[2]) * cc[2];
        }
        double inv[3][3];
        for (int j = 0; j < 3; ++j) {
            double Ac[3][3], e[3] = {0, 0, 0}, col[3];
            for (int r = 0; r < 3; ++r)
                for (int k = 0; k < 3; ++k) Ac[r][k] = A[r][k];
            e[j] = 1.0;
            pais::jacobi_lstsq<3, 3>(Ac, e, col);
            for (int r = 0; r < 3; ++r) inv[r][j] = col[r];
        }
        for (int r = 0; r < 3; ++r) {
            double sacc = 0;
            for (int k = 0; k < 3; ++k) sacc += inv[r][k] * b[k];
            c[r] = sacc;
        }
    }
    const int id = pais_mvs_add_seed(m, c, num_cam, cam_idx);
    if (id >= 0)
        for (int i = 0; i < num_cam; ++i) {
            m->patches[id]->r.imgPoint[i][0] = img_points[2 * i];
            m->patches[id]->r.imgPoint[i][1] = img_points[2 * i + 1];
        }
    return id;
}

#define MHIP(call)                                                                  \
    do {                                                                            \
        hipError_t e__ = (call);                                                    \
        if (e__ != hipSuccess) { g_mvs_err = std::string(#call ": ") + hipGetErrorString(e__); return -2; } \
    } while (0)

static int refine_local(pais_mvs *m, int n, const pais_candidate *c, pais_patch_result *out, int has_seeds,
                        const pais_patch_result **view = nullptr)
{
    if (n <= 0) return 0;
    if (view) *view = out;
    if (m->ctx) {
        int rc = view ? pais_refine_batch_view(m->ctx, n, c, view) : pais_refine_batch(m->ctx, n, c, out);
        if (rc) g_mvs_err = pais_last_error();
        return rc;
    }
    if (m->recordSource) {
        if (m->recordSource(m->recordUser, n, c, out, has_seeds)) return mfail("record source failed");
        return 0;
    }
    return mfail("this driver has neither a GPU context nor a record source");
}

static constexpr size_t kWireHeader = 64;
static int all_gather_host(pais_mvs *m, const void *send, void *recv, size_t bytes)
{
    if (!m->gatherCb) return mfail("no host all-gather installed");
    if (m->gatherCb(m->gatherUser, send, recv, bytes)) return mfail("all-gather callback failed");
    return 0;
}

struct WireHeader { uint32_t magic; int32_t rc; int32_t count; int32_t rank; uint32_t user; };
static bool sharded_transport(const pais_mvs *m) { return m->ctx && (m->nccl || m->emuMode == 2); }
static bool host_transport(const pais_mvs *m) { return !sharded_transport(m) && m->gatherCb != nullptr; }

static int shard_growth_handshake(pais_mvs *m, int localRc)
{
    if (host_transport(m)) {
        std::vector<int> all((size_t)m->world, 0);
        int mine = localRc;
        if (all_gather_host(m, &mine, all.data(), sizeof(int))) return -3;
        for (int r = 0; r < m->world; ++r)
            if (all[(size_t)r] != 0) {
                if (!localRc) g_mvs_err = "sharded batch: rank " + std::to_string(r) + " could not grow its exchange buffers";
                return all[(size_t)r] < 0 ? all[(size_t)r] : -2;
            }
        return 0;
    }
    if (m->emuMode == 2 || !m->nccl) return localRc;
    hipStream_t xs = (hipStream_t)pais_ctx_stream(m->ctx);
    std::string err;
    rccl::Api *a = rccl::api(err);
    if (!a || !m->d_hs) return localRc ? localRc : -2;
    m->h_hs[0] = localRc;
    if (hipMemcpyAsync(m->d_hs, m->h_hs, sizeof(int), hipMemcpyHostToDevice, xs) != hipSuccess) return -2;
    if (a->allGather(m->d_hs, m->d_hsAll, sizeof(int), rccl::kInt8, m->nccl, xs) != 0) return -3;
    if (hipMemcpyAsync(m->h_hs, m->d_hsAll, sizeof(int) * (size_t)m->world, hipMemcpyDeviceToHost, xs) != hipSuccess) return -2;
    if (hipStreamSynchronize(xs) != hipSuccess) return -2;
    for (int r = 0; r < m->world; ++r)
        if (m->h_hs[r] != 0) {
            if (!localRc) g_mvs_err = "sharded batch: rank " + std::to_string(r) + " could not grow its exchange buffers";
            return m->h_hs[r] < 0 ? m->h_hs[r] : -2;
        }
    return 0;
}

static int shard_ensure(pais_mvs *m, pais_mvs::ShardBufs &B, size_t per, size_t slot)
{
    const int world = m->world;
    if (host_transport(m)) {
        const bool grow = per > B.hostC.size() || slot > B.hostS.size() || slot * (size_t)world > B.hostAll.size();
        if (!grow) return 0;
        int rc = 0;
        if (m->injectGrowthFail > 0 && --m->injectGrowthFail == 0) { rc = -2; g_mvs_err = "injected: exchange buffers could not grow"; }
        if (!rc) {
            const size_t cap = per + per / 2 + 64, capS = slot * 3 / 2 + 4096;
            B.hostC.resize(std::max(cap, B.hostC.size()));
            B.hostR.resize(B.hostC.size());
            B.hostS.resize(std::max(capS, B.hostS.size()));
            B.hostAll.resize(std::max(B.hostS.size() * (size_t)world, B.hostAll.size()));
        }
        return shard_growth_handshake(m, rc);
    }
    const bool growShard = per > B.shardCap, growWire = slot * (size_t)world > B.wireCap || slot > B.wireSCap;
    if (!growShard && !growWire && B.packed) return 0;
    hipStream_t xs = (hipStream_t)pais_ctx_stream(m->ctx);
    int rc = 0;
    auto ok = [&](hipError_t e, const char *what) {
        if (e != hipSuccess && !rc) { rc = -2; g_mvs_err = std::string(what) + ": " + hipGetErrorString(e); }
        return e == hipSuccess;
    };
    ok(hipSetDevice(m->device), "hipSetDevice");
    ok(hipDeviceSynchronize(), "hipDeviceSynchronize");
    if (!B.packed) {
// ... 129 lines not shown
    X.per = (n + world - 1) / world;
    X.lo = std::min(m->rank * X.per, n);
    X.cnt = shard_count(m, m->rank, n, X.per);
    X.Kb = 1;
    for (int i = 0; i < n; ++i) X.Kb = std::max(X.Kb, c[i].num_cam);
    X.Kmax = 1;
    for (int j = 0; j < X.cnt; ++j) X.Kmax = std::max(X.Kmax, c[shard_index(m, m->rank, j, n, X.per)].num_cam);
    X.WB = pais_record_wire_bytes(X.Kb);
    X.slot = kWireHeader + X.WB * (size_t)X.per;
    X.t0 = now_ms();
    int rc = shard_ensure(m, B, (size_t)X.per, X.slot);
    if (rc) { X.open = false; return rc; }
    const hipError_t sd = host_transport(m) ? hipSuccess : hipSetDevice(m->device);
    if (m->emuMode == 2 && (rc = emu_fill_blocks(m, X)) != 0) { X.open = false; return rc; }
    if (sd != hipSuccess) g_mvs_err = std::string("hipSetDevice: ") + hipGetErrorString(sd);
    shard_refine_enqueue(m, X, (sd != hipSuccess || preFail) ? -2 : 0);
    rc = shard_exchange(m, X);
    if (rc) X.open = false;
    return rc;
}

static int shard_finish(pais_mvs *m, pais_mvs::ShardXfer &X, pais_patch_result *out)
{
    if (!X.open) return mfail("sharded batch: nothing in flight");
    X.open = false;
    const int world = m->world;
    pais_mvs::ShardBufs &B = *X.B;
    const bool host = host_transport(m);
    const unsigned char *wireAll = host ? B.hostAll.data() : B.h_wireAll;
    for (int attempt = 0;; ++attempt) {
        if (!host) MHIP(hipEventSynchronize(B.done));
        if (m->emuMode == 2 && m->emuLatencyUs > 0) {
            const double t1 = now_ms() + m->emuLatencyUs * 1e-3;
            while (now_ms() < t1) {}
        }
        const int mine = host ? (X.hostRetry ? 1 : 0)
                              : (X.cnt > 0 ? pais_ctx_batch_status(X.lane) : 0);
        bool retry = false;
        for (int r = 0; r < world; ++r) {
            WireHeader hd;
            memcpy(&hd, wireAll + X.slot * (size_t)r, sizeof(hd));
            if (r == 0 && hd.magic == PAIS_WIRE_MAGIC) m->streamAgreed = (hd.user & 1u) != 0;
            const int rcnt = shard_count(m, r, X.n, X.per);
            if (hd.magic != PAIS_WIRE_MAGIC || hd.rank != r || hd.count != rcnt) return mfail("sharded batch: malformed exchange header (ranks disagree on the batch)");
            if (hd.rc == PAIS_WIRE_RC_RING_RETRY) { retry = true; continue; }
            if (hd.rc != 0) {
                if (r != m->rank || g_mvs_err.empty()) g_mvs_err = "sharded batch: rank " + std::to_string(r) + " failed to refine its shard (rc " + std::to_string(hd.rc) + ")";
                return hd.rc < 0 ? hd.rc : -1;
            }
        }
        if (!retry) break;
        if (attempt >= 1) return mfail("sharded batch: a shard did not complete twice");
        X.secondAttempt = true;
        m->st.exchange_retries++;
        if (mine == 1) shard_refine_enqueue(m, X);
        else if (!host && X.lane != m->ctx) MHIP(hipEventRecord(B.packed, (hipStream_t)pais_ctx_stream(X.lane)));
        int rc = shard_exchange(m, X);
        if (rc) return rc;
    }
    m->st.exchange_ms += now_ms() - X.t0;
    for (int r = 0; r < world; ++r) {
        const int rcnt = shard_count(m, r, X.n, X.per);
        const unsigned char *blk = wireAll + X.slot * (size_t)r + kWireHeader;
        if (!m->shardStrided) {
            if (rcnt > 0 && pais_unpack_records(rcnt, blk, X.Kb, out + shard_index(m, r, 0, X.n, X.per))) return mfail(pais_last_error());
        } else {
            for (int j = 0; j < rcnt; ++j)
                if (pais_unpack_records(1, blk + X.WB * (size_t)j, X.Kb, out + shard_index(m, r, j, X.n, X.per))) return mfail(pais_last_error());
        }
    }
    return 0;
}

static void emu_record(pais_mvs *m, int n, const pais_candidate *c, const pais_patch_result *recs)
{
    for (int i = 0; i < n; ++i) {
        auto it = m->emuIndex.find(c[i].key);
        if (it != m->emuIndex.end()) { m->emuRecs[it->second] = recs[i]; continue; }
        m->emuIndex.emplace(c[i].key, (uint32_t)m->emuRecs.size());
        m->emuRecs.push_back(recs[i]);
    }
}

static int refine_any(pais_mvs *m, int n, const pais_candidate *c, pais_patch_result *out, int has_seeds, const pais_patch_result **view)
{
    *view = out;
    if (n <= 0) return 0;
    const int world = m->world;
    if (world <= 1 && !m->nccl && !m->gatherCb) {
        const int rc = refine_local(m, n, c, out, has_seeds, view);
        if (!rc && m->emuMode == 1) emu_record(m, n, c, *view);
        return rc;
    }
    const long wavesPerIter = (long)n * m->cfg.particleNum * (has_seeds ? 2 : 1);
    if (wavesPerIter < (long)m->replicateBelow) {
        m->st.batches_replicated++;
        return refine_local(m, n, c, out, has_seeds, view);
    }
    m->st.batches_sharded++;
    m->results.resize((size_t)n);
    if (!sharded_transport(m) && !host_transport(m)) return mfail("sharded batch: no transport attached");
    int rc = shard_submit(m, m->sx[0], m->sb[0], m->ctx, n, c, has_seeds);
    if (!rc) rc = shard_finish(m, m->sx[0], m->results.data());
    if (rc) return rc;
    *view = m->results.data();
    return 0;
}

extern "C" int pais_mvs_test_inject(pais_mvs *m, int what, int count)
{
    if (!m || count < 0) return mfail("pais_mvs_test_inject: bad argument");
    if (what == 1) m->injectRingRetry = count;
    else if (what == 2) m->injectGrowthFail = count;
    else if (what == 3) m->injectRefineFail = count;
    else return mfail("pais_mvs_test_inject: unknown injection");
    return 0;
}

extern "C" int pais_comm_get_unique_id(pais_unique_id *out)
{
    if (!out) return mfail("pais_comm_get_unique_id: bad argument");
    std::string err;
    rccl::Api *a = rccl::api(err);
    if (!a) return mfail(err.c_str());
    rccl::UniqueId id;
    int nr = a->getUniqueId(&id);
    if (nr != 0) { g_mvs_err = std::string("ncclGetUniqueId: ") + (a->errorString ? a->errorString(nr) : "error"); return -3; }
    memcpy(out->bytes, id.internal, PAIS_UNIQUE_ID_BYTES);
    return 0;
}

extern "C" int pais_mvs_comm_init_rccl(pais_mvs *m, int rank, int world, const pais_unique_id *id)
{
    if (!m || !id || world < 1 || rank < 0 || rank >= world) return mfail("pais_mvs_comm_init_rccl: bad argument");
    if (!m->ctx) return mfail("pais_mvs_comm_init_rccl: this driver owns no GPU");
    if (m->nccl || m->gatherCb) return mfail("pais_mvs_comm_init_rccl: a communicator is already attached");
    std::string err;
    rccl::Api *a = rccl::api(err);
    if (!a) return mfail(err.c_str());
    MHIP(hipSetDevice(m->device));
    rccl::UniqueId uid;
    memcpy(uid.internal, id->bytes, PAIS_UNIQUE_ID_BYTES);
    rccl::Comm comm = nullptr;
    int nr = a->commInitRank(&comm, world, uid, rank);
    if (nr != 0) { g_mvs_err = std::string("ncclCommInitRank: ") + (a->errorString ? a->errorString(nr) : "error"); return -3; }
    m->nccl = comm;
    m->rank = rank;
    m->world = world;
    MHIP(hipMalloc((void **)&m->d_hs, sizeof(int)));
    MHIP(hipMalloc((void **)&m->d_hsAll, sizeof(int) * (size_t)world));
    MHIP(hipHostMalloc((void **)&m->h_hs, sizeof(int) * (size_t)std::max(world, 1), hipHostMallocDefault));
    return 0;
}

extern "C" int pais_mvs_emulate(pais_mvs *m, int mode, int rank, int world)
{
    if (!m || mode < 0 || mode > 2) return mfail("pais_mvs_emulate: bad argument");
    if (m->nccl || m->gatherCb) return mfail("pais_mvs_emulate: a communicator is attached");
    if (mode == 2 && (!m->ctx || world < 1 || rank < 0 || rank >= world)) return mfail("pais_mvs_emulate: bad rank / world, or no GPU");
    if (mode == 2 && m->emuRecs.empty()) return mfail("pais_mvs_emulate: nothing recorded (run the workload in mode 1 first)");
    if (const char *e = getenv("PAIS_EMU_LATENCY_US")) m->emuLatencyUs = atof(e);
    m->emuMode = mode;
    if (mode == 2) { m->rank = rank; m->world = world; }
    else { m->rank = 0; m->world = 1; }
    if (mode == 0) { m->emuIndex.clear(); std::vector<pais_patch_result>().swap(m->emuRecs); }
    return 0;
}

extern "C" int pais_mvs_create_ranked(const pais_config *cfg, int num_cams, const pais_camera_desc *cams, int device,
                                      uint64_t pso_seed, int rank, int world, const pais_unique_id *id, pais_mvs **out)
{
    if (device < 0) return mfail("pais_mvs_create_ranked: a rank needs a GPU");
    int rc = pais_mvs_create(cfg, num_cams, cams, device, pso_seed, out);
    if (rc) return rc;
    rc = pais_mvs_comm_init_rccl(*out, rank, world, id);
    if (rc) { pais_mvs_destroy(*out); *out = nullptr; }
    return rc;
}

extern "C" int pais_mvs_comm_init_callback(pais_mvs *m, int rank, int world, pais_allgather_fn fn, void *user)
{
    if (!m || !fn || world < 1 || rank < 0 || rank >= world) return mfail("pais_mvs_comm_init_callback: bad argument");
    if (m->nccl || m->gatherCb) return mfail("pais_mvs_comm_init_callback: a communicator is already attached");
    m->gatherCb = fn;
    m->gatherUser = user;
    m->rank = rank;
    m->world = world;
    return 0;
// ... 282 lines not shown
    };
    auto prefetchEntries = [&](size_t k, bool patch) {
        if (k >= nAct) return;
        const Target c = m->slotCell(m->patches[m->active[k].id]->r, m->active[k].slot);
        const CellMap &map = m->cellMaps[c.cam];
        for (int j = 0; j < 4; ++j) {
            const Target t = neighbour_cell(c, j);
            if (!map.inMap(t.x, t.y)) continue;
            const CellMap::Cell *cl = map.cell(t.x, t.y);
            if (!cl || cl->head < 0) continue;
            if (m->blocksValid && cl->block < m->curRound) continue;
            const int e = cl->head;
            if (patch) __builtin_prefetch(&m->hot[m->pool[e].id]);
            else __builtin_prefetch(&m->pool[e]);
        }
    };
    for (size_t k = 0; k < 16 && k < nAct; ++k) prefetchRecord(k);
    for (size_t k = 0; k < 8 && k < nAct; ++k) prefetchCells(k);
    for (size_t k = 0; m->deepPrefetch && k < 4 && k < nAct; ++k) prefetchEntries(k, false);
    for (size_t k = 0; m->deepPrefetch && k < 2 && k < nAct; ++k) prefetchEntries(k, true);
    const bool split = nAct >= m->streamAbove && !thin;
    const size_t splitAt = (m->onFirstPart && split) ? (size_t)((double)nAct * m->streamSplit) : (size_t)-1;
    const int nParts = (m->onPart && split) ? stream_part_count(m) : 1;
    auto splitPoint = [&](int k) -> size_t {
        const double f = m->streamFirst > 0 ? m->streamFirst : 1.0 / nParts;
        const double at = f + (1.0 - f) * (double)(k - 1) / (double)(nParts - 1);
        return std::max((size_t)1, std::min(nAct - 1, (size_t)((double)nAct * at)));
    };
    size_t nextSplit = nParts > 1 ? splitPoint(1) : (size_t)-1;
    for (size_t actIdx = 0; actIdx < nAct; ++actIdx) {
        if (actIdx == splitAt) {
            m->firstPart = (int)m->candRecs.size();
            if (m->firstPart > 0 && m->onFirstPart(m->partUser, m->candRecs.data(), m->firstPart)) return -2;
        }
        if (actIdx == nextSplit && actIdx > 0) {
            const int done = m->partEnd.empty() ? 0 : m->partEnd.back(), now = (int)m->candRecs.size();
            const int part = (int)m->partEnd.size();
            m->partEnd.push_back(now);
            if (now > done && m->onPart(m->partUser, part, m->candRecs.data() + done, now - done)) return -2;
            nextSplit = part + 2 >= nParts ? (size_t)-1 : std::max(actIdx + 1, splitPoint(part + 2));
        }
        prefetchRecord(actIdx + 16);
        prefetchCells(actIdx + 8);
        if (m->deepPrefetch) {
            prefetchEntries(actIdx + 4, false);
            prefetchEntries(actIdx + 2, true);
        }
        parent_units(m, m->active[actIdx], thin, consider);
    }
    return 0;
}

extern "C" int pais_mvs_round_begin(pais_mvs *m, int B, const pais_candidate **cands, int *n)
{
    if (!m || !cands || !n) return mfail("pais_mvs_round_begin: bad argument");
    const double t0 = now_ms();
    *cands = nullptr;
    *n = 0;
    m->firstPart = -1;
    top_up_active(m, std::max(B, 1));
    if (m->active.empty() && m->deferred.empty()) return 1;

    m->cands.clear();
    m->candRecs.clear();
    m->nextDeferred.clear();
    m->partEnd.clear();
    const bool thin = (int)m->active.size() <= m->thinFront;
    const bool sharded = m->shardEnum && m->world > 1 && !m->onFirstPart && (host_transport(m) || m->nccl || m->emuMode == 2) &&
                         m->deferred.size() + 4 * m->active.size() >= m->shardEnumAbove;
    const int rc = sharded ? list_sharded(m, thin) : list_plain(m, thin);
    if (rc) return rc;
    if (m->truncatedVisible > 0) {
        m->truncatedVisible = 0;
        return mfail("a candidate's visibility cone holds more than PAIS_MAX_VIS cameras (patch.cpp:723-761 keeps them all): "
                     "this rig needs a larger PAIS_MAX_VIS or a larger visibleCorrelation");
    }
    *cands = m->candRecs.data();
    *n = (int)m->candRecs.size();
    m->lastEnumerateMs = now_ms() - t0;
    m->st.host_enumerate_ms += m->lastEnumerateMs;
    return 0;
}

static void commit_records(pais_mvs *m, const pais_patch_result *results, int q0, int q1)
{
    for (int q = q0; q < q1; ++q) {
        const Candidate &c = m->cands[q];
        const pais_patch_result &pr = m->patches[c.u.id]->r;
        if (m->skipNeighborCell(m->cellMaps[c.cam], c.cx, c.cy, pr, -1)) continue;
        m->st.candidates_effective++;
        m->st.pso_evals_effective += results[q - q0].pso_evals;
        m->insertPatch(results[q - q0]);
    }
}
static int commit_finish(pais_mvs *m, int n);

extern "C" int pais_mvs_round_commit(pais_mvs *m, const pais_patch_result *results, int n)
{
    if (!m || n != (int)m->cands.size() || (n && !results)) return mfail("pais_mvs_round_commit: bad argument");
    double t0 = now_ms();
    commit_records(m, results, 0, n);
    const int rc = commit_finish(m, n);
    m->st.host_commit_ms += now_ms() - t0;
    return rc;
}

static int commit_finish(pais_mvs *m, int n)
{
    size_t w = 0;
    for (size_t a = 0; a < m->active.size(); ++a) {
        Active e = m->active[a];
        e.slot++;
        if (e.slot < m->patches[e.id]->r.num_cam) m->active[w++] = e;
    }
    m->active.resize(w);
    m->deferred.swap(m->nextDeferred);
    m->nextDeferred.clear();
    m->st.candidates_refined += n;
    m->st.rounds++;
    m->curRound++;
    m->cands.clear();
    return 0;
}


extern "C" int pais_mvs_load_patch(pais_mvs *m, const double center[3], const double normalS[2], int num_cam,
                                   const int32_t *cam_idx, double fitness, double correlation)
{
    if (!m || !center || !normalS || num_cam < 0 || num_cam > PAIS_MAX_VIS || (num_cam && !cam_idx))
        return mfail("pais_mvs_load_patch: bad argument");
    pais_patch_result r;
    memset(&r, 0, sizeof(r));
    for (int i = 0; i < 3; ++i) r.center[i] = center[i];
    r.normalS[0] = normalS[0];
    r.normalS[1] = normalS[1];
    pais::spherical2normal(normalS[0], normalS[1], r.normal);
    r.num_cam = num_cam;
    for (int i = 0; i < num_cam; ++i) {
        if (cam_idx[i] < 0 || cam_idx[i] >= (int)m->cams.size()) return mfail("pais_mvs_load_patch: bad camera index");
        r.cam_idx[i] = cam_idx[i];
        m->project0(cam_idx[i], center, r.imgPoint[i]);
    }
    r.type = PAIS_TYPE_SEED;
    r.fitness = fitness;
    r.correlation = correlation;
    r.ref_cam = -1;
    {
        double maxCorr = -DBL_MAX;
        for (int i = 0; i < num_cam; ++i) {
            const HostCamera &cam = m->cams[cam_idx[i]];
            const double corr = r.normal[0] * (-cam.optN[0]) + r.normal[1] * (-cam.optN[1]) + r.normal[2] * (-cam.optN[2]);
            if (corr > maxCorr) { maxCorr = corr; r.ref_cam = cam_idx[i]; }
        }
    }
    r.lod = -1;
    r.key = (uint64_t)m->patches.size();
    const int id = m->storePatch(r);
    m->patches[id]->expanded = true;
    return id;
}

extern "C" int pais_mvs_load_patches(pais_mvs *m, int n, const pais_loaded_patch *patches, int *first_id)
{
    if (!m || n < 0 || (n && !patches)) return mfail("pais_mvs_load_patches: bad argument");
    if (!m->ctx)
        return mfail("pais_mvs_load_patches: this driver was created without a GPU context (the loader state is a HIP kernel; there is no host path)");
    if (first_id) *first_id = (int)m->patches.size();
    if (n == 0) return 0;
    std::vector<pais_patch_result> recs((size_t)n);
    if (pais_load_state_batch(m->ctx, n, patches, recs.data())) return mfail(pais_last_error());
    for (int i = 0; i < n; ++i) {
        recs[i].key = (uint64_t)m->patches.size();
        m->storePatch(recs[i]);
    }
    return 0;
}

static void filter_prepare(pais_mvs *m)
{
    if (m->cellMaps.empty()) {
        m->setNeighborRadius();
        m->setCellMaps();
    }
}
static void cell_ids(const pais_mvs *m, const CellMap &map, int x, int y, std::vector<int> &out)
{
    out.clear();
// ... 244 lines not shown
    {
        pais_mvs::ShardXfer &X = m->sx[idx];
        if (!X.open) return 0;
        if (X.sharded) { *view = out; return shard_finish(m, X, out); }
        X.open = false;
        const int rc = pais_refine_batch_end(X.lane, view);
        if (rc) g_mvs_err = pais_last_error();
        return rc;
    }
    pais_ctx *part_lane(int p)
    {
        if (p == 0) return m->ctx;
        while ((int)m->partLanes.size() < p) {
            pais_ctx *l = nullptr;
            if (pais_ctx_fork_lane(m->ctx, &l)) { g_mvs_err = pais_last_error(); laneForkFailed = true; return m->ctx; }
            m->partLanes.push_back(l);
        }
        return m->partLanes[p - 1];
    }
    void drain_parts(int from, int to)
    {
        const pais_patch_result *dummy;
        m->results.resize(std::max((size_t)1, m->candRecs.size()));
        for (int p = from; p < to; ++p) (void)part_finish(p, m->results.data(), &dummy);
    }
    int next_part(int part, const pais_candidate *cc, int np)
    {
        const double t = now_ms();
        if (partsOut == 0) tFirst = t;
        pais_ctx *lane = part_lane(part);
        beginRc = lane ? part_submit(part, lane, np, cc, np * stream_part_count(m)) : -2;
        partsOut = part + 1;
        enqueueMs += now_ms() - t;
        return beginRc;
    }
    int first_part(const pais_candidate *cc, int n0)
    {
        tFirst = now_ms();
        (void)pais_ctx_set_round_hint(m->ctx, (int)((double)n0 / m->streamSplit));
        beginRc = pais_refine_batch_open(m->ctx, n0, cc, m->streamHead);
        if (beginRc) g_mvs_err = pais_last_error();
        enqueueMs = now_ms() - tFirst;
        return beginRc;
    }
    static int on_part(void *self, int part, const pais_candidate *cc, int np) { return ((RoundStream *)self)->next_part(part, cc, np); }
    static int on_first_part(void *self, const pais_candidate *cc, int n0) { return ((RoundStream *)self)->first_part(cc, n0); }
};

struct RoundTimes {
    double refineMs = 0;
    double commitMs = 0;
};

static int round_sharded_parts(pais_mvs *m, RoundStream &rs, const pais_candidate *c, int n, bool canaryRound, RoundTimes *T)
{
    m->results.resize((size_t)std::max(n, 1));
    std::vector<int> ends(m->partEnd);
    ends.push_back(n);
    const int P = (int)ends.size();
    for (int p = 0; p < P; ++p) m->sx[p].c = c + (p ? ends[p - 1] : 0);
    {
        const int lo = ends[P - 2], np = n - lo;
        if (np > 0) {
            if (rs.partsOut == 0) rs.tFirst = now_ms();
            pais_ctx *lane = rs.part_lane(P - 1);
            if (!lane || rs.part_submit(P - 1, lane, np, c + lo, n)) { rs.drain_parts(0, rs.partsOut); return -2; }
            rs.partsOut = P;
        }
    }
    const bool canary = canaryRound && n > 0;
    if (canary) m->canaryRecs.resize((size_t)n);
    pais_patch_result *out = canary ? m->canaryRecs.data() : m->results.data();
    double commitMs = 0;
    for (int p = 0; p < P; ++p) {
        const int lo = p ? ends[p - 1] : 0, np = ends[p] - lo;
        if (np <= 0) continue;
        const pais_patch_result *v = nullptr;
        if (rs.part_finish(p, out + lo, &v)) { rs.drain_parts(p + 1, P); return -2; }
        if (canary) {
            if (v != out + lo) memcpy(out + lo, v, sizeof(pais_patch_result) * (size_t)np);
            continue;
        }
        const double t1 = now_ms();
        commit_records(m, v, lo, ends[p]);
        commitMs += now_ms() - t1;
    }
    if (canary) {
        int rc2 = shard_submit(m, m->sx[0], m->sb[0], m->ctx, n, c, 0);
        if (!rc2) rc2 = shard_finish(m, m->sx[0], m->results.data());
        if (rc2) return rc2;
        const bool same = memcmp(m->canaryRecs.data(), m->results.data(), sizeof(pais_patch_result) * (size_t)n) == 0;
        const int verdict = shard_growth_handshake(m, same ? 0 : -7);
        m->streamCanary = verdict ? -1 : 1;
        if (getenv("PAIS_STREAM_CANARY_LOG"))
            fprintf(stderr, "[pais] rank %d: streamed sharded round of %d candidates in %d parts %s its unstreamed replay -> streaming %s\n",
                    m->rank, n, P, same ? "==" : "!=", m->streamCanary > 0 ? "on" : "off");
        const double t1 = now_ms();
        commit_records(m, m->results.data(), 0, n);
        commitMs += now_ms() - t1;
    }
    const double t2 = now_ms();
    const int rc = commit_finish(m, n);
    commitMs += now_ms() - t2;
    m->st.host_commit_ms += commitMs;
    T->commitMs = commitMs;
    T->refineMs = n > 0 ? std::max(0.0, (now_ms() - rs.tFirst) - commitMs) : 0.0;
    return rc;
}

static int round_two_lanes(pais_mvs *m, RoundStream &rs, const pais_candidate *c, int n, RoundTimes *T)
{
    const int n0 = m->firstPart, n1 = n - n0;
    const pais_patch_result *dummy;
    if (n1 > 0) {
        if (!m->lane1 && pais_ctx_fork_lane(m->ctx, &m->lane1)) { g_mvs_err = pais_last_error(); return -2; }
        if (n0 == 0) rs.tFirst = now_ms();
        (void)pais_ctx_set_round_hint(m->lane1, n);
        if (pais_refine_batch_open(m->lane1, n1, c + n0, m->streamHead)) {
            g_mvs_err = pais_last_error();
            if (n0 > 0) (void)pais_refine_batch_end(m->ctx, &dummy);
            return -2;
        }
    }
    for (int a = n0 > 0 ? 0 : 1, b = n1 > 0 ? 0 : 1; !a || !b;) {
        if (!a) a = pais_refine_batch_enqueue(m->ctx, m->streamStep);
        if (!b && a >= 0) b = pais_refine_batch_enqueue(m->lane1, m->streamStep);
        if (a < 0 || b < 0) {
            g_mvs_err = pais_last_error();
            if (a >= 0 && n0 > 0) (void)pais_refine_batch_end(m->ctx, &dummy);
            if (b >= 0 && n1 > 0) (void)pais_refine_batch_end(m->lane1, &dummy);
            return -2;
        }
    }
    double commitMs = 0;
    const pais_patch_result *v0 = nullptr, *v1 = nullptr;
    if (n0 > 0) {
        if (pais_refine_batch_end(m->ctx, &v0)) {
            g_mvs_err = pais_last_error();
            if (n1 > 0) (void)pais_refine_batch_end(m->lane1, &v1);
            return -2;
        }
        const double t1 = now_ms();
        commit_records(m, v0, 0, n0);
        commitMs += now_ms() - t1;
    }
    if (n1 > 0 && pais_refine_batch_end(m->lane1, &v1)) { g_mvs_err = pais_last_error(); return -2; }
    const double t2 = now_ms();
    if (n1 > 0) commit_records(m, v1, n0, n);
    const int rc = commit_finish(m, n);
    commitMs += now_ms() - t2;
    m->st.host_commit_ms += commitMs;
    T->commitMs = commitMs;
    T->refineMs = n > 0 ? std::max(0.0, (now_ms() - rs.tFirst) - commitMs) : 0.0;
    return rc;
}

static int round_one_batch(pais_mvs *m, const pais_candidate *c, int n, RoundTimes *T, int *sharded)
{
    m->results.resize((size_t)(n > 0 ? n : 1));
    const pais_patch_result *recs = m->results.data();
    const int64_t shardedBefore = m->st.batches_sharded;
    if (n > 0) {
        const double t0 = now_ms();
        const int rc = refine_any(m, n, c, m->results.data(), 0, &recs);
        T->refineMs = now_ms() - t0;
        if (rc) return rc;
    }
    *sharded = m->st.batches_sharded > shardedBefore ? 1 : 0;
    const double t1 = now_ms();
    const int rc = pais_mvs_round_commit(m, recs, n);
    T->commitMs = now_ms() - t1;
    return rc;
}

static int finish_round(pais_mvs *m, int n, int kmax, int sharded, bool streamed, double tRef, double enumMs, double commitMs)
{
    m->st.gpu_refine_ms += tRef;
    if (streamed) m->st.rounds_streamed++;
    if (n > 0) m->roundLog.push_back(pais_round_log{n, 0, sharded, kmax, tRef, enumMs, commitMs});
    m->prevHostMs = enumMs + commitMs;
    m->prevGpuMs = streamed ? tRef + commitMs : tRef;
    return checkpoint_after_round(m);
}

extern "C" int pais_mvs_expansion_patches(pais_mvs *m, int B, int max_rounds)
{
    if (!m || (!m->ctx && !m->recordSource)) return mfail("pais_mvs_expansion_patches: no GPU context");
    int rc = pais_mvs_expansion_begin(m);
    if (rc) return rc;
    m->ckptCalls = 0;
    for (int rounds = 0;;) {
        const StreamChoice sc = stream_choice(m);
        RoundStream rs{m};
        const pais_candidate *c;
        int n;
        m->partUser = &rs;
        m->onFirstPart = (sc.canStream && !sc.shardStream) ? RoundStream::on_first_part : nullptr;
        m->onPart = (sc.canStream && sc.shardStream) ? RoundStream::on_part : nullptr;
        rc = pais_mvs_round_begin(m, B, &c, &n);
        m->onFirstPart = nullptr;
        m->onPart = nullptr;
        m->partUser = nullptr;
        m->lastEnumerateMs -= rs.enqueueMs;
        m->st.host_enumerate_ms -= rs.enqueueMs;
        if (rc < 0) {
            const pais_patch_result *dummy;
            if (sc.shardStream) rs.drain_parts(0, rs.partsOut);
            else if (m->firstPart > 0 && !rs.beginRc) (void)pais_refine_batch_end(m->ctx, &dummy);
            m->firstPart = -1;
            return rs.beginRc ? rs.beginRc : rc;
        }
        if (rc == 1) { if (sc.shardStream) rs.drain_parts(0, rs.partsOut); break; }
        const double enumMs = m->lastEnumerateMs;
        int kmax = 1;
        for (int i = 0; i < n; ++i) kmax = std::max(kmax, c[i].num_cam);
        RoundTimes T;
        const bool parts = sc.shardStream && !m->partEnd.empty(), streamed = parts || m->firstPart >= 0;
        int sharded = parts ? 1 : 0;
        if (parts) rc = round_sharded_parts(m, rs, c, n, sc.canaryRound, &T);
        else if (streamed) rc = round_two_lanes(m, rs, c, n, &T);
        else rc = round_one_batch(m, c, n, &T, &sharded);
        if (rc) return rc;
        if ((rc = finish_round(m, n, kmax, sharded, streamed, T.refineMs, enumMs, T.commitMs))) return rc;
        if (max_rounds > 0 && ++rounds >= max_rounds) break;
    }
    return pais_mvs_expansion_end(m);
}

extern "C" int pais_mvs_seeds_from_matches(pais_mvs *m, int num_cams, const pais_keypoints *kp, int num_matches,
                                           const pais_pair_match *matches, double max_dist, int *num_seeds)
{
    if (!m || !kp || num_cams != (int)m->cams.size() || num_matches < 0 || (num_matches && !matches))
        return mfail("pais_mvs_seeds_from_matches: bad argument");
    const int C = num_cams;
    for (int c = 0; c < C; ++c)
        if (kp[c].n < 0 || (kp[c].n && !kp[c].xy)) return mfail("pais_mvs_seeds_from_matches: bad keypoints");
    std::vector<double> Fs((size_t)C * C * 9, 0.0);
    {
        std::vector<pais_camera_desc> d((size_t)C);
        for (int c = 0; c < C; ++c) {
            memset(&d[c], 0, sizeof(pais_camera_desc));
            memcpy(d[c].KR, m->cams[c].KR, sizeof(d[c].KR));
            memcpy(d[c].KT, m->cams[c].KT, sizeof(d[c].KT));
            memcpy(d[c].center, m->cams[c].C, sizeof(d[c].center));
        }
        for (int i = 0; i < C; ++i)
            for (int j = i; j < C; ++j) {
                double *Fij = &Fs[((size_t)i * C + j) * 9], *Fji = &Fs[((size_t)j * C + i) * 9];
                if (i == j) { Fij[0] = Fij[4] = Fij[8] = 1.0; continue; }
                if (pais_seed_fundamental(&d[j], &d[i], Fij)) return mfail(pais_seed_last_error());
                for (int r = 0; r < 3; ++r)
                    for (int c = 0; c < 3; ++c) Fji[r * 3 + c] = Fij[c * 3 + r];
            }
// ... 199 lines not shown
```

Baseline: 203,900.

## Copy compact wire records device-to-host instead of full patch result structs

The final after-kernel phase now packs each patch result into a compact wire slot on device that keeps only the header fields and the per-camera arrays up to Kmax. The host copies this packed buffer instead of the full fixed-size pais_patch_result array. The commit path reads records through a view that unpacks each slot lazily. This cuts PCIe transfer volume and pinned host memory per round, at the cost of extra device stores and per-record unpacking on the host.

```diff
diff --git a/include/pais_hip.h b/include/pais_hip.h
--- a/include/pais_hip.h
+++ b/include/pais_hip.h
@@ -198,6 +198,8 @@
 int  pais_pack_records(int n, const pais_patch_result *recs, int max_num_cam, void *wire);
 int  pais_unpack_records(int n, const void *wire, int max_num_cam, pais_patch_result *recs);
 int  pais_pack_records_device(pais_ctx *ctx, int n, const pais_patch_result *d_recs, int max_num_cam, void *d_wire);
+int  pais_refine_batch_view_wire(pais_ctx *ctx, int n, const pais_candidate *cands, const void **wire, int *max_num_cam);
+int  pais_refine_batch_end_wire(pais_ctx *ctx, const void **wire, int *max_num_cam);
 
 #define PAIS_WIRE_MAGIC 0x50414953u
 #define PAIS_WIRE_RC_RING_RETRY 1
diff --git a/pais_mvs_amd/_lib.py b/pais_mvs_amd/_lib.py
--- a/pais_mvs_amd/_lib.py
+++ b/pais_mvs_amd/_lib.py
@@ -184,6 +184,13 @@
     L.pais_refine_batch_enqueue.argtypes = [C.c_void_p, C.c_int]
     L.pais_ctx_set_round_hint.argtypes = [C.c_void_p, C.c_int]
     L.pais_refine_batch_end.argtypes = [C.c_void_p, C.POINTER(C.POINTER(PatchResult))]
+    L.pais_record_wire_bytes.restype = C.c_size_t
+    L.pais_record_wire_bytes.argtypes = [C.c_int]
+    L.pais_pack_records.argtypes = [C.c_int, C.POINTER(PatchResult), C.c_int, C.c_void_p]
+    L.pais_unpack_records.argtypes = [C.c_int, C.c_void_p, C.c_int, C.POINTER(PatchResult)]
+    L.pais_pack_records_device.argtypes = [C.c_void_p, C.c_int, C.c_void_p, C.c_int, C.c_void_p]
+    L.pais_refine_batch_view_wire.argtypes = [C.c_void_p, C.c_int, C.POINTER(Candidate), C.POINTER(C.c_void_p), C.POINTER(C.c_int)]
+    L.pais_refine_batch_end_wire.argtypes = [C.c_void_p, C.POINTER(C.c_void_p), C.POINTER(C.c_int)]
     L.pais_ctx_fork_lane.argtypes = [C.c_void_p, C.POINTER(C.c_void_p)]
     L.pais_get_kernel_stats.argtypes = [C.c_void_p, C.POINTER(KernelStats), C.c_int]
     L.pais_ctx_set_fine_timing.argtypes = [C.c_void_p, C.c_int]
diff --git a/pais_mvs_amd/context.py b/pais_mvs_amd/context.py
--- a/pais_mvs_amd/context.py
+++ b/pais_mvs_amd/context.py
@@ -96,6 +96,15 @@
         _lib.check(self.L.pais_refine_batch(self.h, n, arr, out), "pais_refine_batch")
         return out
 
+    def refine_batch_wire(self, cands: Sequence["_lib.Candidate"]):
+        n = len(cands)
+        arr = (_lib.Candidate * max(n, 1))(*cands)
+        wire, kmax = C.c_void_p(), C.c_int(0)
+        _lib.check(self.L.pais_refine_batch_view_wire(self.h, n, arr, C.byref(wire), C.byref(kmax)), "pais_refine_batch_view_wire")
+        if n == 0:
+            return b"", 0
+        return C.string_at(wire, self.L.pais_record_wire_bytes(kmax.value) * n), kmax.value
+
     def ncc_batch(self, states: Sequence["_lib.ViewState"], tables: bool = False) -> "NccBatch":
         n = len(states)
         arr = (_lib.ViewState * max(n, 1))(*states)
diff --git a/pais_mvs_amd/csrc/pais_capi.hip b/pais_mvs_amd/csrc/pais_capi.hip
--- a/pais_mvs_amd/csrc/pais_capi.hip
+++ b/pais_mvs_amd/csrc/pais_capi.hip
@@ -89,6 +89,8 @@
     Slice sl[16];
     int *cnt = nullptr, *nextCnt = nullptr;
     const pais_candidate *d_cands = nullptr;
+    void *wire = nullptr;
+    int wireKw = 0;
     Timed tp;
     TraceOut *trace = nullptr;
 };
@@ -110,7 +112,10 @@
     DevBuf<pais_candidate> d_cands;
     DevBuf<pais_patch_result> d_recs;
     PinBuf<pais_candidate> h_cands;
-    PinBuf<pais_patch_result> h_recs;
+    DevBuf<unsigned char> d_wire;
+    PinBuf<unsigned char> h_wire;
+    int wireMaxCam = 1;
+    std::vector<pais_patch_result> h_recs;
     DevBuf<double> d_hp;
     DevBuf<double> d_ratios;
     DevBuf<int> d_counters;
@@ -1089,12 +1094,20 @@
     ctx->psoLaunches++;
     Timed ta;
     if (ta.begin(ctx, ctx->stream, &ctx->evAfter)) return -2;
-    HIPCHK(pais_launch::after(sc, P.all.recs, P.all.n, ctx->d_hp, P.afterGrid, P.cnt, ctx->stat, P.all.Kmax, ctx->d_ratios, P.nextCnt, ctx->stream));
+    HIPCHK(pais_launch::after(sc, P.all.recs, P.all.n, ctx->d_hp, P.afterGrid, P.cnt, ctx->stat, P.all.Kmax, ctx->d_ratios, P.nextCnt, P.wire, P.wireKw,
+                              ctx->stream));
     if (ta.end()) return -2;
     return 0;
 }
 
-static int batch_setup(pais_ctx *ctx, PassPlan &P, int n, const pais_candidate *d_cands, pais_patch_result *d_out, int max_num_cam, int has_seeds)
+struct WireOut {
+    void *d_wire = nullptr;
+    int maxCam = 1;
+};
+static inline int wire_kw(int max_num_cam);
+
+static int batch_setup(pais_ctx *ctx, PassPlan &P, int n, const pais_candidate *d_cands, pais_patch_result *d_out, int max_num_cam, int has_seeds,
+                       const WireOut &w)
 {
     HIPCHK(hipSetDevice(ctx->device));
     const DevScene &sc = ctx->sc;
@@ -1121,6 +1134,8 @@
     P.hasSeeds = has_seeds != 0;
     P.afterGrid = afterGrid;
     P.d_cands = d_cands;
+    P.wire = w.d_wire;
+    P.wireKw = wire_kw(w.maxCam);
 
     if (ctx->countersDirty) HIPCHK(hipMemsetAsync(ctx->d_counters, 0, sizeof(int) * 8, ctx->stream));
     ctx->countersDirty = true;
@@ -1145,13 +1160,13 @@
 }
 
 static int refine_device_once(pais_ctx *ctx, int n, const pais_candidate *d_cands, pais_patch_result *d_out, int max_num_cam, int has_seeds,
-                              bool defer = false, TraceOut *trace = nullptr)
+                              const WireOut &w, bool defer = false, TraceOut *trace = nullptr)
 {
     PassPlan &P = ctx->plan;
     P.trace = trace;
     ctx->ringUsed = false;
     ctx->ringPendingN = 0;
-    int rc = batch_setup(ctx, P, n, d_cands, d_out, max_num_cam, has_seeds);
+    int rc = batch_setup(ctx, P, n, d_cands, d_out, max_num_cam, has_seeds, w);
     int againCount = 0;
     const int maxPass = has_seeds ? (PAIS_MAX_VIS + 2) : 1;
     for (int pass = 0; !rc && pass < maxPass; ++pass) {
@@ -1173,21 +1188,22 @@
 }
 
 static int rerun_without_ring(pais_ctx *ctx, int n, const pais_candidate *d_cands, pais_patch_result *d_out, int max_num_cam, int has_seeds,
-                              bool defer, int hint)
+                              const WireOut &w, bool defer, int hint)
 {
     ctx->ringSuppressed = true;
     ctx->countersDirty = true;
     ctx->roundHint = hint;
-    const int rc = refine_device_once(ctx, n, d_cands, d_out, max_num_cam, has_seeds, defer);
+    const int rc = refine_device_once(ctx, n, d_cands, d_out, max_num_cam, has_seeds, w, defer);
     ctx->ringSuppressed = false;
     return rc;
 }
 
-static int refine_device(pais_ctx *ctx, int n, const pais_candidate *d_cands, pais_patch_result *d_out, int max_num_cam, int has_seeds, bool defer)
+static int refine_device(pais_ctx *ctx, int n, const pais_candidate *d_cands, pais_patch_result *d_out, int max_num_cam, int has_seeds,
+                         const WireOut &w, bool defer)
 {
     const int hint = ctx->roundHint;
-    const int rc = refine_device_once(ctx, n, d_cands, d_out, max_num_cam, has_seeds, defer);
-    return rc == 1 ? rerun_without_ring(ctx, n, d_cands, d_out, max_num_cam, has_seeds, defer, hint) : rc;
+    const int rc = refine_device_once(ctx, n, d_cands, d_out, max_num_cam, has_seeds, w, defer);
+    return rc == 1 ? rerun_without_ring(ctx, n, d_cands, d_out, max_num_cam, has_seeds, w, defer, hint) : rc;
 }
 
 extern "C" int pais_refine_batch_device(pais_ctx *ctx, int n, const pais_candidate *d_cands, pais_patch_result *d_out,
@@ -1197,7 +1213,7 @@
     if (n == 0) return 0;
     if (!d_cands || !d_out) return fail_msg("pais_refine_batch_device: null pointer");
     if (ctx->openBatch >= 0) return fail_msg("pais_refine_batch_device: a batch is open on this context");
-    return refine_device(ctx, n, d_cands, d_out, max_num_cam, has_seeds, false);
+    return refine_device(ctx, n, d_cands, d_out, max_num_cam, has_seeds, WireOut{}, false);
 }
 
 extern "C" int pais_refine_batch_device_async(pais_ctx *ctx, int n, const pais_candidate *d_cands, pais_patch_result *d_out,
@@ -1209,9 +1225,9 @@
     if (ctx->openBatch >= 0) return fail_msg("pais_refine_batch_device_async: a batch is open on this context");
     if (ctx->ringSuppressOnce) {
         ctx->ringSuppressOnce = false;
-        return rerun_without_ring(ctx, n, d_cands, d_out, max_num_cam, has_seeds, true, ctx->roundHint);
-    }
-    return refine_device(ctx, n, d_cands, d_out, max_num_cam, has_seeds, true);
+        return rerun_without_ring(ctx, n, d_cands, d_out, max_num_cam, has_seeds, WireOut{}, true, ctx->roundHint);
+    }
+    return refine_device(ctx, n, d_cands, d_out, max_num_cam, has_seeds, WireOut{}, true);
 }
 
 extern "C" int pais_ctx_batch_status(pais_ctx *ctx)
@@ -1249,6 +1265,11 @@
     return 0;
 }
 
+static hipError_t wire_copy_down(pais_ctx *ctx, int n)
+{
+    return hipMemcpyAsync(ctx->h_wire, ctx->d_wire, pais_record_wire_bytes(ctx->wireMaxCam) * (size_t)n, hipMemcpyDeviceToHost, ctx->stream);
+}
+
 extern "C" int pais_refine_batch_view(pais_ctx *ctx, int n, const pais_candidate *cands, const pais_patch_result **view)
 {
     if (!ctx || n < 0) return fail_msg("pais_refine_batch: bad argument");
@@ -1257,6 +1278,16 @@
     int rc = pais_refine_batch_begin(ctx, n, cands);
     if (rc) return rc;
     return pais_refine_batch_end(ctx, view);
+}
+
+extern "C" int pais_refine_batch_view_wire(pais_ctx *ctx, int n, const pais_candidate *cands, const void **wire, int *max_num_cam)
+{
+    if (!ctx || n < 0) return fail_msg("pais_refine_batch_view_wire: bad argument");
+    if (n == 0) return 0;
+    if (!cands || !wire || !max_num_cam) return fail_msg("pais_refine_batch_view_wire: null pointer");
+    int rc = pais_refine_batch_begin(ctx, n, cands);
+    if (rc) return rc;
+    return pais_refine_batch_end_wire(ctx, wire, max_num_cam);
 }
 
 extern "C" int pais_refine_batch_begin(pais_ctx *ctx, int n, const pais_candidate *cands)
@@ -1280,15 +1311,13 @@
     if (!rc) rc = pass_close(ctx, P);
     if (rc) { (void)pass_join(ctx, P); ctx->openBatch = -1; ctx->ringUsed = false; return rc; }
     ctx->countersDirty = false;
-    HIPCHK(hipMemcpyAsync(ctx->h_recs, ctx->d_recs, sizeof(pais_patch_result) * (size_t)ctx->openBatch, hipMemcpyDeviceToHost, ctx->stream));
+    HIPCHK(wire_copy_down(ctx, ctx->openBatch));
     ctx->planDone = true;
     return 1;
 }
 
-extern "C" int pais_refine_batch_end(pais_ctx *ctx, const pais_patch_result **view)
-{
-    if (!ctx || !view) return fail_msg("pais_refine_batch_end: bad argument");
-    if (ctx->openBatch < 0) return fail_msg("pais_refine_batch_end: no batch is open on this context");
+static int batch_end_slots(pais_ctx *ctx, int *nOut)
+{
     if (!ctx->planDone) {
         const int rc = pais_refine_batch_enqueue(ctx, 0);
         if (rc < 0) return rc;
@@ -1298,12 +1327,37 @@
     HIPCHK(hipStreamSynchronize(ctx->stream));
     if (ring_failed(ctx, ctx->plan.all.n)) {
         const int n = ctx->plan.all.n;
-        const int rc = rerun_without_ring(ctx, n, ctx->d_cands, ctx->d_recs, ctx->plan.all.Kmax, 0, false, ctx->roundHint);
+        const int rc = rerun_without_ring(ctx, n, ctx->d_cands, ctx->d_recs, ctx->plan.all.Kmax, 0, WireOut{ctx->d_wire, ctx->wireMaxCam}, false, ctx->roundHint);
         if (rc) return rc;
-        HIPCHK(hipMemcpyAsync(ctx->h_recs, ctx->d_recs, sizeof(pais_patch_result) * (size_t)n, hipMemcpyDeviceToHost, ctx->stream));
+        HIPCHK(wire_copy_down(ctx, n));
         HIPCHK(hipStreamSynchronize(ctx->stream));
     }
-    *view = ctx->h_recs;
+    *nOut = ctx->plan.all.n;
+    return 0;
+}
+
+extern "C" int pais_refine_batch_end(pais_ctx *ctx, const pais_patch_result **view)
+{
+    if (!ctx || !view) return fail_msg("pais_refine_batch_end: bad argument");
+    if (ctx->openBatch < 0) return fail_msg("pais_refine_batch_end: no batch is open on this context");
+    int n = 0;
+    const int rc = batch_end_slots(ctx, &n);
+    if (rc) return rc;
+    if (ctx->h_recs.size() < (size_t)n) ctx->h_recs.resize((size_t)n);
+    if (pais_unpack_records(n, ctx->h_wire, ctx->wireMaxCam, ctx->h_recs.data())) return -1;
+    *view = ctx->h_recs.data();
+    return 0;
+}
+
+extern "C" int pais_refine_batch_end_wire(pais_ctx *ctx, const void **wire, int *max_num_cam)
+{
+    if (!ctx || !wire || !max_num_cam) return fail_msg("pais_refine_batch_end_wire: bad argument");
+    if (ctx->openBatch < 0) return fail_msg("pais_refine_batch_end_wire: no batch is open on this context");
+    int n = 0;
+    const int rc = batch_end_slots(ctx, &n);
+    if (rc) return rc;
+    *wire = ctx->h_wire;
+    *max_num_cam = ctx->wireMaxCam;
     return 0;
 }
 
@@ -1319,19 +1373,22 @@
     HIPCHK(ctx->d_cands.reserve(ctx->stream, sizeof(pais_candidate) * (size_t)n));
     HIPCHK(ctx->d_recs.reserve(ctx->stream, sizeof(pais_patch_result) * (size_t)n));
     HIPCHK(ctx->h_cands.reserve(ctx->stream, sizeof(pais_candidate) * (size_t)n));
-    HIPCHK(ctx->h_recs.reserve(ctx->stream, sizeof(pais_patch_result) * (size_t)n));
+    HIPCHK(ctx->d_wire.reserve(ctx->stream, pais_record_wire_bytes(Kmax) * (size_t)n));
+    HIPCHK(ctx->h_wire.reserve(ctx->stream, pais_record_wire_bytes(Kmax) * (size_t)n));
+    ctx->wireMaxCam = Kmax;
+    const WireOut w{ctx->d_wire, Kmax};
     memcpy(ctx->h_cands, cands, sizeof(pais_candidate) * (size_t)n);
     HIPCHK(hipMemcpyAsync(ctx->d_cands, ctx->h_cands, sizeof(pais_candidate) * (size_t)n, hipMemcpyHostToDevice, ctx->stream));
     if (hasSeeds) {
-        rc = pais_refine_batch_device(ctx, n, ctx->d_cands, ctx->d_recs, Kmax, 1);
+        rc = refine_device(ctx, n, ctx->d_cands, ctx->d_recs, Kmax, 1, w, false);
         if (rc) return rc;
-        HIPCHK(hipMemcpyAsync(ctx->h_recs, ctx->d_recs, sizeof(pais_patch_result) * (size_t)n, hipMemcpyDeviceToHost, ctx->stream));
+        HIPCHK(wire_copy_down(ctx, n));
         ctx->openBatch = n;
         ctx->planDone = true;
         return 0;
     }
     PassPlan &P = ctx->plan;
-    rc = batch_setup(ctx, P, n, ctx->d_cands, ctx->d_recs, Kmax, 0);
+    rc = batch_setup(ctx, P, n, ctx->d_cands, ctx->d_recs, Kmax, 0, w);
     if (!rc) rc = pass_open(ctx, P, 0, 0);
     ctx->roundHint = 0;
     if (!rc && (rc = pass_iterations(ctx, P, iterations > 0 ? iterations : 0)) != 0) (void)pass_join(ctx, P);
@@ -1440,7 +1497,7 @@
         if (particles) HIPCHK(hipMemsetAsync(ctx->d_tParts, 0, sizeof(double) * 11 * nRuns * rows * NP, ctx->stream));
         TraceOut t;
         t.sink = pais_launch::TraceSink{ctx->d_tRuns, ctx->d_tIters, particles ? ctx->d_tParts.p : nullptr, max_runs, rows};
-        rc = refine_device_once(ctx, m, ctx->d_tCands, ctx->d_tRecs, Kmax, hasSeeds, false, &t);
+        rc = refine_device_once(ctx, m, ctx->d_tCands, ctx->d_tRecs, Kmax, hasSeeds, WireOut{}, false, &t);
         if (rc) {
             (void)hipStreamSynchronize(ctx->stream);
             return rc < 0 ? rc : fail_msg("pais_pso_trace: unexpected ring pass");
diff --git a/pais_mvs_amd/csrc/pais_internal.h b/pais_mvs_amd/csrc/pais_internal.h
--- a/pais_mvs_amd/csrc/pais_internal.h
+++ b/pais_mvs_amd/csrc/pais_internal.h
@@ -103,7 +103,7 @@
                     int phase, unsigned long long timeoutTicks);
 void ring_profile_print();
 hipError_t after(const DevScene &sc, pais_patch_result *recs, int n, double *hpScratch, int grid, int *counters,
-                 unsigned long long *stat, int Kmax, double *ratios, int *nextCounters, hipStream_t stream);
+                 unsigned long long *stat, int Kmax, double *ratios, int *nextCounters, void *wire, int wireKw, hipStream_t stream);
 size_t ncc_lds_bytes(int Kmax);
 bool hp_in_lds(const DevScene &sc, int Kmax);
 hipError_t ncc_batch(const DevScene &sc, const pais_view_state *states, int n, pais_view_result *out, double *tables, int stride,
diff --git a/pais_mvs_amd/csrc/pais_kernels.hip b/pais_mvs_amd/csrc/pais_kernels.hip
--- a/pais_mvs_amd/csrc/pais_kernels.hip
+++ b/pais_mvs_amd/csrc/pais_kernels.hip
@@ -1977,10 +1977,26 @@
     ratios[(size_t)c * PAIS_MAX_VIS + k] = region_ratio(pt[0], pt[1], sc.cfg.patchRadius, H);
 }
 
+__device__ __forceinline__ int wire_src_word(int w, int Kw)
+{
+    if (w < 34) return w;
+    if (w < 36) return 290 + (w - 34);
+    if (w < 44) return 292 + (w - 36);
+    if (w < 52) return 364 + (w - 44);
+    if (w < 52 + 4 * Kw) return 34 + (w - 52);
+    return 300 + (w - 52 - 4 * Kw);
+}
+__device__ __forceinline__ void store_wire_slot(uint32_t *wire, int c, int Kw, const pais_patch_result *src, int tid, int nthreads)
+{
+    const int wordsPerSlot = 52 + 5 * Kw;
+    uint32_t *dst = wire + (size_t)c * wordsPerSlot;
+    for (int w = tid; w < wordsPerSlot; w += nthreads) dst[w] = ((const uint32_t *)src)[wire_src_word(w, Kw)];
+}
+
 template <int PHASE>
 __global__ __launch_bounds__(64 * AFTER_WAVES) void k_after(DevScene sc, pais_patch_result *recs, int n, double *hpScratch,
                                                               int *counters, unsigned long long *stat, int Kmax, double *ratios,
-                                                              int hpInLds, int *nextCounters)
+                                                              int hpInLds, int *nextCounters, uint32_t *wire, int wireKw)
 {
     if (PHASE == 2 && nextCounters && blockIdx.x == 0 && threadIdx.x == 0) {
         nextCounters[0] = 0;
@@ -1999,8 +2015,10 @@
     double *hp = hpInLds ? (double *)(smem + off) : hpScratch + (size_t)blockIdx.x * Kmax * S2;
     for (int c = blockIdx.x; c < n; c += gridDim.x) {
         const int stg = recs[c].stage;
-        if (PHASE == 1 ? (stg != PAIS_STAGE_AFTER) : (stg != PAIS_STAGE_AFTER2 && stg != PAIS_STAGE_AFTER2_KEEP && stg != PAIS_STAGE_AFTER2_SAME))
+        if (PHASE == 1 ? (stg != PAIS_STAGE_AFTER) : (stg != PAIS_STAGE_AFTER2 && stg != PAIS_STAGE_AFTER2_KEEP && stg != PAIS_STAGE_AFTER2_SAME)) {
+            if (PHASE == 2 && wire) store_wire_slot(wire, c, wireKw, &recs[c], threadIdx.x, 64 * AFTER_WAVES);
             continue;
+        }
         __syncthreads();
         copy_record(st, &recs[c], threadIdx.x, 64 * AFTER_WAVES);
         __syncthreads();
@@ -2093,6 +2111,7 @@
         }
         __syncthreads();
         copy_record(&recs[c], st, threadIdx.x, 64 * AFTER_WAVES);
+        if (PHASE == 2 && wire) store_wire_slot(wire, c, wireKw, st, threadIdx.x, 64 * AFTER_WAVES);
     }
 }
 
@@ -2192,13 +2211,7 @@
     for (size_t t = (size_t)blockIdx.x * 256 + threadIdx.x; t < (size_t)n * wordsPerSlot; t += (size_t)gridDim.x * 256) {
         const int r = (int)(t / wordsPerSlot), w = (int)(t - (size_t)r * wordsPerSlot);
         const uint32_t *src = (const uint32_t *)&recs[r];
-        int sw;
-        if (w < 34) sw = w;
-        else if (w < 36) sw = 290 + (w - 34);
-        else if (w < 44) sw = 292 + (w - 36);
-        else if (w < 52) sw = 364 + (w - 44);
-        else if (w < 52 + 4 * Kw) sw = 34 + (w - 52);
-        else sw = 300 + (w - 52 - 4 * Kw);
+        const int sw = wire_src_word(w, Kw);
         wire[t] = src[sw];
     }
 }
@@ -2547,7 +2560,7 @@
 }
 
 hipError_t after(const DevScene &sc, pais_patch_result *recs, int n, double *hpScratch, int grid, int *counters,
-                 unsigned long long *stat, int Kmax, double *ratios, int *nextCounters, hipStream_t stream)
+                 unsigned long long *stat, int Kmax, double *ratios, int *nextCounters, void *wire, int wireKw, hipStream_t stream)
 {
     if (n <= 0) return hipSuccess;
     const int hpInLds = hp_in_lds(sc, Kmax) ? 1 : 0;
@@ -2555,10 +2568,10 @@
     const dim3 rgrid((unsigned)(((long)n * Kmax + 63) / 64)), block(64 * AFTER_WAVES);
     hipError_t e = launch<k_region_ratio>(rgrid, dim3(64), 0, stream, sc, recs, n, PAIS_STAGE_AFTER, ratios, Kmax);
     if (e == hipSuccess)
-        e = launch<k_after<1>>(dim3(grid), block, lds, stream, sc, recs, n, hpScratch, counters, stat, Kmax, ratios, hpInLds, (int *)nullptr);
+        e = launch<k_after<1>>(dim3(grid), block, lds, stream, sc, recs, n, hpScratch, counters, stat, Kmax, ratios, hpInLds, (int *)nullptr, (uint32_t *)nullptr, 0);
     if (e == hipSuccess) e = launch<k_region_ratio>(rgrid, dim3(64), 0, stream, sc, recs, n, PAIS_STAGE_AFTER2, ratios, Kmax);
     if (e == hipSuccess)
-        e = launch<k_after<2>>(dim3(grid), block, lds, stream, sc, recs, n, hpScratch, counters, stat, Kmax, ratios, hpInLds, nextCounters);
+        e = launch<k_after<2>>(dim3(grid), block, lds, stream, sc, recs, n, hpScratch, counters, stat, Kmax, ratios, hpInLds, nextCounters, (uint32_t *)wire, wireKw);
     return e;
 }
 hipError_t ncc_batch(const DevScene &sc, const pais_view_state *states, int n, pais_view_result *out, double *tables, int stride,
diff --git a/pais_mvs_amd/csrc/pais_mvs.hip b/pais_mvs_amd/csrc/pais_mvs.hip
--- a/pais_mvs_amd/csrc/pais_mvs.hip
+++ b/pais_mvs_amd/csrc/pais_mvs.hip
@@ -886,11 +886,44 @@
         if (e__ != hipSuccess) { g_mvs_err = std::string(#call ": ") + hipGetErrorString(e__); return -2; } \
     } while (0)
 
+struct RecView {
+    const pais_patch_result *full = nullptr;
+    const unsigned char *wire = nullptr;
+    int maxCam = 0;
+    RecView() = default;
+    explicit RecView(const pais_patch_result *f) : full(f) {}
+    RecView(const void *w, int k) : wire((const unsigned char *)w), maxCam(k) {}
+    const pais_patch_result &record(int i, pais_patch_result *tmp) const
+    {
+        if (!wire) return full[i];
+        const int Kw = (std::max(1, std::min(maxCam, (int)PAIS_MAX_VIS)) + 1) & ~1;
+        const unsigned char *w = wire + pais_record_wire_bytes(maxCam) * (size_t)i;
+        unsigned char *r = (unsigned char *)tmp;
+        memcpy(r, w, 136);
+        memcpy(r + 1160, w + 136, 8);
+        memcpy(r + 1168, w + 144, 32);
+        memcpy(r + 1456, w + 176, 32);
+        const int K = std::max(0, std::min(tmp->num_cam, Kw));
+        memcpy(r + 136, w + 208, 16 * (size_t)K);
+        memcpy(r + 1200, w + 208 + 16 * (size_t)Kw, 4 * (size_t)K);
+        return *tmp;
+    }
+};
+
 static int refine_local(pais_mvs *m, int n, const pais_candidate *c, pais_patch_result *out, int has_seeds,
-                        const pais_patch_result **view = nullptr)
+                        const pais_patch_result **view = nullptr, RecView *slots = nullptr)
 {
     if (n <= 0) return 0;
     if (view) *view = out;
+    if (m->ctx && view && slots) {
+        const void *w = nullptr;
+        int maxCam = 0;
+        const int rc = pais_refine_batch_view_wire(m->ctx, n, c, &w, &maxCam);
+        if (rc) g_mvs_err = pais_last_error();
+        *slots = RecView(w, maxCam);
+        *view = nullptr;
+        return rc;
+    }
     if (m->ctx) {
         int rc = view ? pais_refine_batch_view(m->ctx, n, c, view) : pais_refine_batch(m->ctx, n, c, out);
         if (rc) g_mvs_err = pais_last_error();
@@ -1186,20 +1219,25 @@
     }
 }
 
-static int refine_any(pais_mvs *m, int n, const pais_candidate *c, pais_patch_result *out, int has_seeds, const pais_patch_result **view)
+static int refine_any(pais_mvs *m, int n, const pais_candidate *c, pais_patch_result *out, int has_seeds, const pais_patch_result **view,
+                      RecView *slots = nullptr)
 {
     *view = out;
+    if (slots) *slots = RecView(out);
     if (n <= 0) return 0;
     const int world = m->world;
     if (world <= 1 && !m->nccl && !m->gatherCb) {
-        const int rc = refine_local(m, n, c, out, has_seeds, view);
+        const int rc = refine_local(m, n, c, out, has_seeds, view, m->emuMode == 1 ? nullptr : slots);
         if (!rc && m->emuMode == 1) emu_record(m, n, c, *view);
+        if (slots && *view) *slots = RecView(*view);
         return rc;
     }
     const long wavesPerIter = (long)n * m->cfg.particleNum * (has_seeds ? 2 : 1);
     if (wavesPerIter < (long)m->replicateBelow) {
         m->st.batches_replicated++;
-        return refine_local(m, n, c, out, has_seeds, view);
+        const int rc = refine_local(m, n, c, out, has_seeds, view, slots);
+        if (slots && *view) *slots = RecView(*view);
+        return rc;
     }
     m->st.batches_sharded++;
     m->results.resize((size_t)n);
@@ -1208,6 +1246,7 @@
     if (!rc) rc = shard_finish(m, m->sx[0], m->results.data());
     if (rc) return rc;
     *view = m->results.data();
+    if (slots) *slots = RecView(*view);
     return 0;
 }
 
@@ -1656,27 +1695,34 @@
     return 0;
 }
 
-static void commit_records(pais_mvs *m, const pais_patch_result *results, int q0, int q1)
-{
+static void commit_records(pais_mvs *m, const RecView &results, int q0, int q1)
+{
+    pais_patch_result slot;
     for (int q = q0; q < q1; ++q) {
         const Candidate &c = m->cands[q];
         const pais_patch_result &pr = m->patches[c.u.id]->r;
         if (m->skipNeighborCell(m->cellMaps[c.cam], c.cx, c.cy, pr, -1)) continue;
+        const pais_patch_result &r = results.record(q - q0, &slot);
         m->st.candidates_effective++;
-        m->st.pso_evals_effective += results[q - q0].pso_evals;
-        m->insertPatch(results[q - q0]);
+        m->st.pso_evals_effective += r.pso_evals;
+        m->insertPatch(r);
     }
 }
 static int commit_finish(pais_mvs *m, int n);
 
-extern "C" int pais_mvs_round_commit(pais_mvs *m, const pais_patch_result *results, int n)
-{
-    if (!m || n != (int)m->cands.size() || (n && !results)) return mfail("pais_mvs_round_commit: bad argument");
+static int round_commit(pais_mvs *m, const RecView &results, int n)
+{
     double t0 = now_ms();
     commit_records(m, results, 0, n);
     const int rc = commit_finish(m, n);
     m->st.host_commit_ms += now_ms() - t0;
     return rc;
+}
+
+extern "C" int pais_mvs_round_commit(pais_mvs *m, const pais_patch_result *results, int n)
+{
+    if (!m || n != (int)m->cands.size() || (n && !results)) return mfail("pais_mvs_round_commit: bad argument");
+    return round_commit(m, RecView{results}, n);
 }
 
 static int commit_finish(pais_mvs *m, int n)
@@ -2087,7 +2133,7 @@
             continue;
         }
         const double t1 = now_ms();
-        commit_records(m, v, lo, ends[p]);
+        commit_records(m, RecView(v), lo, ends[p]);
         commitMs += now_ms() - t1;
     }
     if (canary) {
@@ -2101,7 +2147,7 @@
             fprintf(stderr, "[pais] rank %d: streamed sharded round of %d candidates in %d parts %s its unstreamed replay -> streaming %s\n",
                     m->rank, n, P, same ? "==" : "!=", m->streamCanary > 0 ? "on" : "off");
         const double t1 = now_ms();
-        commit_records(m, m->results.data(), 0, n);
+        commit_records(m, RecView(m->results.data()), 0, n);
         commitMs += now_ms() - t1;
     }
     const double t2 = now_ms();
@@ -2138,20 +2184,21 @@
         }
     }
     double commitMs = 0;
-    const pais_patch_result *v0 = nullptr, *v1 = nullptr;
+    const void *v0 = nullptr, *v1 = nullptr;
+    int k0 = 0, k1 = 0;
     if (n0 > 0) {
-        if (pais_refine_batch_end(m->ctx, &v0)) {
+        if (pais_refine_batch_end_wire(m->ctx, &v0, &k0)) {
             g_mvs_err = pais_last_error();
-            if (n1 > 0) (void)pais_refine_batch_end(m->lane1, &v1);
+            if (n1 > 0) (void)pais_refine_batch_end(m->lane1, &dummy);
             return -2;
         }
         const double t1 = now_ms();
-        commit_records(m, v0, 0, n0);
+        commit_records(m, RecView(v0, k0), 0, n0);
         commitMs += now_ms() - t1;
     }
-    if (n1 > 0 && pais_refine_batch_end(m->lane1, &v1)) { g_mvs_err = pais_last_error(); return -2; }
+    if (n1 > 0 && pais_refine_batch_end_wire(m->lane1, &v1, &k1)) { g_mvs_err = pais_last_error(); return -2; }
     const double t2 = now_ms();
-    if (n1 > 0) commit_records(m, v1, n0, n);
+    if (n1 > 0) commit_records(m, RecView(v1, k1), n0, n);
     const int rc = commit_finish(m, n);
     commitMs += now_ms() - t2;
     m->st.host_commit_ms += commitMs;
@@ -2164,16 +2211,17 @@
 {
     m->results.resize((size_t)(n > 0 ? n : 1));
     const pais_patch_result *recs = m->results.data();
+    RecView slots(recs);
     const int64_t shardedBefore = m->st.batches_sharded;
     if (n > 0) {
         const double t0 = now_ms();
-        const int rc = refine_any(m, n, c, m->results.data(), 0, &recs);
+        const int rc = refine_any(m, n, c, m->results.data(), 0, &recs, &slots);
         T->refineMs = now_ms() - t0;
         if (rc) return rc;
     }
     *sharded = m->st.batches_sharded > shardedBefore ? 1 : 0;
     const double t1 = now_ms();
-    const int rc = pais_mvs_round_commit(m, recs, n);
+    const int rc = round_commit(m, slots, n);
     T->commitMs = now_ms() - t1;
     return rc;
 }
```

Result: no change. 207,500, median of 6 (+1.8%).
